# dfki-asr/morphablegraphs

Measured on AMD Instinct MI355X. Metric: motion-primitive samples scored+back-projected/sec; fraction of HBM roofline, higher is better.
Workload: dtype f32; 1 GPU; walk primitive L=40 F=156 D=79 NB=31 GMM k=8, batch=8192 candidates/GPU (BASELINE.json configs[1]); candidates_per_gpu=8192, global_candidates=8192, collective=none, clock_ramp_steps=1500

## Files before the change

### morphablegraphs_amd/csrc/mg_frames.hip

```cpp
#include "mg_frames_common.h"

int mg_setup_kernel_attributes(mg_context *) {
    int rc = mg_frames_ws_attributes();
    return rc != MG_OK ? rc : mg_frames_cs_attributes();
}

bool mg_frames_root_split(const mg_primitive *p) {
    const int want = p->ctx->opt[MG_OPT_ROOT_MODE];
    return want == 2 || (want == 3 && p->root_split);
}

static int mg_fused_gmm_lds(const mg_primitive *p) { return 4 * p->K * 16 * 8; }
static int mg_fused_gmm_lds_cs(const mg_primitive *p) {
    const int JT = (int)((p->Lg + 15) / 16);
    return mg_fused_gmm_lds(p) + 2 * p->KK * 64 * 4 + (p->K * JT * 16 + (p->K + 1) / 2 * 2) * 8;
}

static bool mg_fused_gmm_staged(const mg_primitive *p, const mg_time_grid *g) { return g->cs_lds_bytes + mg_fused_gmm_lds_cs(p) <= 160 * 1024; }

bool mg_frames_can_fuse_gmm(const mg_primitive *p, const mg_time_grid *g, int64_t B) {
    const int64_t n_tiles = (B + MG_NCAND - 1) / MG_NCAND;
    const int64_t grid = std::min<int64_t>(n_tiles * g->n_chunks, std::max(1, p->ctx->n_cu - p->ctx->reserved_cus));
    return g->mfma_ok && p->d_gPpack != nullptr && p->K <= 16 && p->KK <= MG_FUSE_MAX_KK && p->Lg == p->L &&
           g->lds_bytes + mg_fused_gmm_lds(p) <= 160 * 1024 &&
           (n_tiles + grid - 1) / grid <= 4;
}

int mg_frames_kernel_choice(const mg_primitive *p, const mg_time_grid *g, int64_t B, bool fused, const void *out, bool lat_f64) {
    const int64_t n_tiles = (B + MG_NCAND - 1) / MG_NCAND;
    const int64_t units = n_tiles * g->n_chunks;
    const int64_t grid0 = std::min<int64_t>(units, std::max(1, p->ctx->n_cu - p->ctx->reserved_cus));
    const int64_t grid_cs = grid0 / g->n_chunks * g->n_chunks;
    const int want = p->ctx->opt[MG_OPT_FRAMES_KERNEL];
    bool cs = g->cs_ok && grid_cs >= g->n_chunks && grid_cs <= 4096 &&
              (!fused || (g->cs_lds_bytes + mg_fused_gmm_lds(p) <= 160 * 1024 && (n_tiles + grid_cs - 1) / grid_cs <= 4));
    const bool cs_spills = p->KK >= 16 || (lat_f64 && p->KK >= 14);
    if (want == 2 && !cs) return -1;
    if (want == 1) cs = false;
    else if (want == 0 && cs_spills) cs = false;
    else if (want == 0) cs = cs && units >= 2 * grid0 && mg_output_class(p->ctx, out) != 0;
    return cs ? 2 : 1;
}
int mg_frames_grid(const mg_primitive *p, const mg_time_grid *g, int64_t B, int which) {
    const int64_t units = (B + MG_NCAND - 1) / MG_NCAND * g->n_chunks;
    const int64_t grid0 = std::min<int64_t>(units, std::max(1, p->ctx->n_cu - p->ctx->reserved_cus));
    return (int)(which == 2 ? grid0 / g->n_chunks * g->n_chunks : grid0);
}

int mg_frames_lds_bytes(const mg_primitive *p, const mg_time_grid *g, int which, bool fused) {
    if (which == 2) return g->cs_lds_bytes + (fused ? (mg_fused_gmm_staged(p, g) ? mg_fused_gmm_lds_cs(p) : mg_fused_gmm_lds(p)) : 0);
    return g->lds_bytes + (fused ? mg_fused_gmm_lds(p) : 0);
}

int mg_launch_frames_mfma(mg_primitive *p, const mg_time_grid *g, const void *lat, int ldt, int64_t B, int64_t ld, float *out, float *logp,
                          int prof_slot, int prof_slot2) {
    mg_frames_args a;
    a.rt_total = p->RT;
    a.B = B; a.ld = ld; a.T = g->T; a.D = p->D; a.Dp = p->Dp; a.cshift = p->cshift; a.L = p->L; a.nroot = p->nroot;
    a.n_chunks = g->n_chunks; a.stride = g->stride; a.max_wi = g->max_wi; a.max_nt = g->max_nt; a.nbuf = g->nbuf;
    const int64_t n_tiles = (B + MG_NCAND - 1) / MG_NCAND;
    const int64_t units = n_tiles * g->n_chunks;
    if (n_tiles >= ((int64_t)1 << 27) || units >= ((int64_t)1 << 31)) {
        mg_set_error("mg_back_project_frames: batch too large for one launch");
        return MG_ERR_UNSUPPORTED;
    }
    a.n_tiles = (int32_t)n_tiles;
    a.max_tiles = g->max_tiles;
    for (int i = 0; i < MG_ARG_CHUNKS; i++) a.ck[i] = i < g->n_chunks ? g->chunks[i] : mg_chunk{};
    a.cs_magic = a.cs_per = a.cs_rem = 0;
    const bool lf = (ldt == MG_F64);
    const int which = mg_frames_kernel_choice(p, g, B, logp != nullptr, out, lf);
    if (which < 0) {
        mg_set_error("mg_back_project_frames: the chunk-stationary kernel does not cover this shape (window of %d row tiles, %d bytes of LDS)",
                     g->max_tiles, g->cs_lds_bytes);
        return MG_ERR_UNSUPPORTED;
    }
    const bool cs = which == 2;
    const int buf_bytes = (MG_NCAND * g->stride * 4 + 255) / 256 * 256;
    int lds = g->nbuf * (buf_bytes + MG_RO_BYTES_N(g->max_nt) + MG_TB_BYTES_N(g->max_nt)) + MG_NCAND * (g->max_wi * p->nroot + 1) * 8 + 128;
    if (lds != g->lds_bytes || lds > 160 * 1024 || (logp && !mg_frames_can_fuse_gmm(p, g, B))) {
        mg_set_error("mg_back_project_frames: internal LDS sizing mismatch (%d vs %d)", lds, g->lds_bytes);
        return MG_ERR_UNSUPPORTED;
    }
    if (cs) lds = g->cs_lds_bytes;
    a.gmm_staged = cs && logp && mg_fused_gmm_staged(p, g) ? 1 : 0;
    if (logp) lds += a.gmm_staged ? mg_fused_gmm_lds_cs(p) : mg_fused_gmm_lds(p);
    const int grid = mg_frames_grid(p, g, B, which);
    if (cs) {
        const int Q = grid / g->n_chunks;
        a.cs_magic = (1 << 20) / g->n_chunks + 1;
        a.cs_per = (int32_t)(n_tiles / Q);
        a.cs_rem = (int32_t)(n_tiles % Q);
    }
    mg_launch_events ev;
    if (prof_slot >= 0) (void)mg_prof_kernel(p->ctx, prof_slot, prof_slot2, &ev.start, &ev.stop);
    const bool split = mg_frames_root_split(p);
    return cs ? mg_launch_frames_cs(p, g, lat, out, logp, a, lf, split, buf_bytes, lds, grid, ev)
              : mg_launch_frames_ws(p, g, lat, out, logp, a, lf, split, buf_bytes, lds, grid, ev);
}
```

### morphablegraphs_amd/csrc/mg_frames_common.h

```cpp
#pragma once
#include "mg_internal.h"
#include <hip/hip_ext.h>
#include <type_traits>
#include "mg_gmm_device.h"

typedef float f32x4 __attribute__((ext_vector_type(4)));
typedef double f64x4 __attribute__((ext_vector_type(4)));
typedef float f32x4u __attribute__((ext_vector_type(4), aligned(4)));
typedef float f32x3u __attribute__((ext_vector_type(3), aligned(4)));
typedef float f32x2u __attribute__((ext_vector_type(2), aligned(4)));

struct mg_frames_args {
    int64_t B, ld;
    int32_t T, D, Dp, cshift, L, nroot, n_chunks, n_tiles, stride, max_wi, max_nt;
    int32_t nbuf;
    int32_t max_tiles;
    int32_t rt_total;
    int32_t gmm_staged;
    int32_t cs_magic, cs_per, cs_rem;
    mg_chunk ck[MG_ARG_CHUNKS];
};

template <bool F64>
__device__ __forceinline__ double mg_load_lat(const void *lat, int64_t idx) {
// ... 153 lines not shown
        *(f32x4u *)op = v;
    } else if (n == 3) {
        f32x3u t = {v[0], v[1], v[2]};
        *(f32x3u *)op = t;
    } else if (n == 2) {
        f32x2u t = {v[0], v[1]};
        *(f32x2u *)op = t;
    } else if (n == 1) {
        op[0] = v[0];
    }
}


template <int KK>
__device__ __forceinline__ void mg_produce_f32(const float2 *__restrict__ ep, const float *__restrict__ mean32,
                                               const mg_chunk &ck, float *lds_c, int stride, int t_first, int pw, int npw,
                                               const float (&sfrag)[KK], int lane, int cl, int g, int rot = 0) {
    float2 fa[2][KK / 2], na[2][KK / 2];
    f32x4 fm[2], nm[2];
    auto load_tile = [&](int t, float2(&fr)[KK / 2], f32x4 &cin) {
        const int tc = t < ck.ntiles ? t : ck.ntiles - 1;
        const float2 *p = ep + ((size_t)(ck.rt0 + tc) * (KK / 2)) * 64 + lane;
#pragma unroll
        for (int q = 0; q < KK / 2; q++) fr[q] = p[q * 64];
        cin = *(const f32x4 *)(mean32 + (size_t)(ck.rt0 + tc) * 16 + 4 * g);
    };
    const int span = ck.ntiles - t_first - pw;
    const int nrounds = span > 0 ? (span + 2 * npw - 1) / (2 * npw) : 0;
    if (nrounds == 0) return;
    int rr = rot % nrounds;
    int t = t_first + pw + 2 * npw * rr;
    load_tile(t, fa[0], fm[0]);
    load_tile(t + npw, fa[1], fm[1]);
    for (int r = 0; r < nrounds; r++) {
        if (++rr == nrounds) rr = 0;
        const int tn = t_first + pw + 2 * npw * rr;
        load_tile(tn, na[0], nm[0]);
        load_tile(tn + npw, na[1], nm[1]);
        f32x4 acc0 = fm[0], acc1 = fm[1];
#pragma unroll
        for (int q = 0; q < KK / 2; q++) {
            acc0 = __builtin_amdgcn_mfma_f32_16x16x4f32(fa[0][q].x, sfrag[2 * q], acc0, 0, 0, 0);
            acc1 = __builtin_amdgcn_mfma_f32_16x16x4f32(fa[1][q].x, sfrag[2 * q], acc1, 0, 0, 0);
            acc0 = __builtin_amdgcn_mfma_f32_16x16x4f32(fa[0][q].y, sfrag[2 * q + 1], acc0, 0, 0, 0);
            acc1 = __builtin_amdgcn_mfma_f32_16x16x4f32(fa[1][q].y, sfrag[2 * q + 1], acc1, 0, 0, 0);
        }
        if (t < ck.ntiles) *(f32x4 *)&lds_c[cl * stride + t * 16 + 4 * g] = acc0;
        if (t + npw < ck.ntiles) *(f32x4 *)&lds_c[cl * stride + (t + npw) * 16 + 4 * g] = acc1;
#pragma unroll
        for (int q = 0; q < KK / 2; q++) { fa[0][q] = na[0][q]; fa[1][q] = na[1][q]; }
        fm[0] = nm[0]; fm[1] = nm[1];
        t = tn;
    }
}

template <int KK, bool LAT_F64>
__device__ __forceinline__ void mg_load_sfrag(float (&sfrag)[KK], const void *lat, const mg_unit &un, int64_t ld, int L, int cl, int g) {
    typename mg_gmm_xt<LAT_F64>::type x[KK];
    mg_gmm_load_x<KK, LAT_F64>(x, lat, un.b0, un.ncand, ld, L, cl, g);
#pragma unroll
    for (int kk = 0; kk < KK; kk++) sfrag[kk] = (float)x[kk];
}


template <int KK, bool LAT_F64>
__device__ __forceinline__ void mg_fused_gmm_terms(mg_lds_int *prog, const double *__restrict__ gPpack,
                                                   const double *__restrict__ gmP, const double *__restrict__ gcst,
                                                   const void *__restrict__ lat, int64_t B, int64_t ld, int L, int n_tiles,
                                                   int gK, int gJT, int pw, int lane, int group) {
    const int cl = lane & 15, g = lane >> 4;
    mg_lds_f64 *gterms = (mg_lds_f64 *)(prog + 32);
    const int64_t gt0 = (int64_t)blockIdx.x * n_tiles / gridDim.x + 2 * group;
    const int64_t gt1 = ((int64_t)blockIdx.x + 1) * n_tiles / gridDim.x;
    if (gt0 < gt1) {
        const bool has_b = gt0 + 1 < gt1;
        typename mg_gmm_xt<LAT_F64>::type xa[KK], xb[KK];
        {
            const int64_t ba = gt0 * MG_NCAND, bb = (has_b ? gt0 + 1 : gt0) * MG_NCAND;
            const int na = (int)((B - ba) < MG_NCAND ? (B - ba) : MG_NCAND);
            const int nb = (int)((B - bb) < MG_NCAND ? (B - bb) : MG_NCAND);
            mg_gmm_load_x<KK, LAT_F64>(xa, lat, ba, na, ld, L, cl, g);
            mg_gmm_load_x<KK, LAT_F64>(xb, lat, bb, nb, ld, L, cl, g);
        }
        for (int k = pw; k < gK; k += MG_WS_NPW) {
            mg_gmm_frag<KK> f;
            mg_gmm_load_component<KK>(f, gPpack, gmP, gcst, k, gJT, lane, cl, gK);
            mg_gmm_apply_component(f, k, gJT, xa, gterms, cl, g);
            if (has_b) mg_gmm_apply_component(f, k, gJT, xb, gterms + gK * 16, cl, g);
        }
    }
    mg_publish(prog + 16, pw, lane, group + 1);
}

template <int KK>
__device__ __forceinline__ void mg_fused_gmm_terms_ldsx(mg_lds_int *prog, const double *__restrict__ gPpack, const mg_lds_f32 *gx, const mg_lds_f64 *mpl,
                                                        const mg_lds_f64 *cstl, int n_tiles, int gK, int gJT, int pw, int lane, bool early) {
    const int cl = lane & 15, g = lane >> 4;
    mg_lds_f64 *gterms = (mg_lds_f64 *)(prog + 32);
    const int64_t gt0 = (int64_t)blockIdx.x * n_tiles / gridDim.x;
    const int64_t gt1 = ((int64_t)blockIdx.x + 1) * n_tiles / gridDim.x;
    if (gt0 < gt1) {
        const bool has_b = gt0 + 1 < gt1;
        int ks[4], nk = 0;
        for (int k = pw; k < gK; k += MG_WS_NPW)
            if (!(early && k >= MG_WS_NPW && k < 2 * MG_WS_NPW)) ks[nk++] = k;
        for (int i = 0; i < nk; i += 2) {
            const int k = ks[i], k2 = i + 1 < nk ? ks[i + 1] : gK;
            mg_gmm_frag<KK> f, f2;
            mg_gmm_load_pf2<KK>(f, gPpack, gK, k, gJT, lane);
            if (k2 < gK) mg_gmm_load_pf2<KK>(f2, gPpack, gK, k2, gJT, lane);
            mg_gmm_apply_component_ldsx<KK>(f, k, gJT, gx, lane, mpl, cstl, gterms, cl, g);
            if (has_b) mg_gmm_apply_component_ldsx<KK>(f, k, gJT, gx + KK * 64, lane, mpl, cstl, gterms + gK * 16, cl, g);
            if (k2 < gK) {
                mg_gmm_apply_component_ldsx<KK>(f2, k2, gJT, gx, lane, mpl, cstl, gterms, cl, g);
                if (has_b) mg_gmm_apply_component_ldsx<KK>(f2, k2, gJT, gx + KK * 64, lane, mpl, cstl, gterms + gK * 16, cl, g);
            }
        }
    }
    mg_publish(prog + 16, pw, lane, 1);
}

template <int KK>
__device__ __forceinline__ void mg_fused_gmm_early_component(mg_lds_int *prog, const mg_gmm_frag<KK> &f, int k, const mg_lds_f32 *gx, const mg_lds_f64 *mpl,
                                                             const mg_lds_f64 *cstl, int n_tiles, int gK, int gJT, int lane) {
    const int cl = lane & 15, g = lane >> 4;
    mg_lds_f64 *gterms = (mg_lds_f64 *)(prog + 32);
    const int64_t gt0 = (int64_t)blockIdx.x * n_tiles / gridDim.x;
    const int64_t gt1 = ((int64_t)blockIdx.x + 1) * n_tiles / gridDim.x;
    mg_gmm_apply_component_ldsx<KK>(f, k, gJT, gx, lane, mpl, cstl, gterms, cl, g);
    if (gt0 + 1 < gt1) mg_gmm_apply_component_ldsx<KK>(f, k, gJT, gx + KK * 64, lane, mpl, cstl, gterms + gK * 16, cl, g);
}

__device__ __forceinline__ void mg_fused_gmm_finish(mg_lds_int *prog, float *__restrict__ logp, int64_t B, int n_tiles, int gK,
                                                    int pw, int lane, int group) {
    mg_lds_int *gdone = prog + 16;
    mg_lds_f64 *gterms = (mg_lds_f64 *)(prog + 32);
    mg_lds_f64 *gexps = gterms + 2 * gK * 16;
    const int64_t gt0 = (int64_t)blockIdx.x * n_tiles / gridDim.x + 2 * group;
    const int64_t gt1 = ((int64_t)blockIdx.x + 1) * n_tiles / gridDim.x;
    if (pw < 2 && gt0 + pw < gt1) {
        mg_wait_producers(gdone, group + 1);
        const mg_lds_f64 *terms = gterms + pw * gK * 16;
        mg_lds_f64 *exps = gexps + pw * gK * 16;
        for (int e = lane; e < gK * 16; e += 64) exps[e] = mg_gmm_exp_entry(terms, gK, e);
        asm volatile("s_waitcnt lgkmcnt(0)" ::: "memory");
        const int64_t b0 = (gt0 + pw) * MG_NCAND;
        if (lane < MG_NCAND && b0 + lane < B) logp[b0 + lane] = (float)mg_gmm_logsumexp(terms, exps, gK, lane);
    }
    if (pw < 2) mg_publish(prog + 24, pw, lane, group + 1);
}


struct mg_launch_events { hipEvent_t start = nullptr, stop = nullptr; };
int mg_launch_frames_ws(mg_primitive *p, const mg_time_grid *g, const void *lat, float *out, float *logp, const mg_frames_args &a, bool lat_f64,
                        bool split, int buf_bytes, int lds, int grid, const mg_launch_events &ev);
int mg_launch_frames_cs(mg_primitive *p, const mg_time_grid *g, const void *lat, float *out, float *logp, const mg_frames_args &a, bool lat_f64,
                        bool split, int buf_bytes, int lds, int grid, const mg_launch_events &ev);
int mg_frames_ws_attributes();
int mg_frames_cs_attributes();
```

### morphablegraphs_amd/csrc/mg_frames_cs.hip

```cpp
#include "mg_frames_common.h"

#define MG_CS_NPW 4
#define MG_CS_NCW 8
#define MG_CS_NSP 4
#define MG_CS_BLOCK (64 * (MG_CS_NPW + MG_CS_NCW))
template <int KK> struct mg_cs_cfg {
    static constexpr int TPWP = 120 / KK < 17 ? 120 / KK : 17;
    static constexpr int TPWS_REGS = 160 / MG_CS_NSP;
    static constexpr int TPWS = TPWS_REGS / KK < 5 ? (TPWS_REGS / KK > 0 ? TPWS_REGS / KK : 1) : 5;
    static constexpr int MAX_TILES = (MG_CS_NPW - 1) * TPWP + MG_CS_NSP * TPWS;
};
int mg_cs_max_tiles(int KK) {
    switch (KK) {
        case 2: return mg_cs_cfg<2>::MAX_TILES;   case 4: return mg_cs_cfg<4>::MAX_TILES;   case 6: return mg_cs_cfg<6>::MAX_TILES;
        case 8: return mg_cs_cfg<8>::MAX_TILES;   case 10: return mg_cs_cfg<10>::MAX_TILES; case 12: return mg_cs_cfg<12>::MAX_TILES;
        case 14: return mg_cs_cfg<14>::MAX_TILES; case 16: return mg_cs_cfg<16>::MAX_TILES; default: return 0;
    }
}

#define MG_CS_PROG_LAT 12
#define MG_CS_PROG_SWEPT 16
#define MG_CS_PROG_MEAN 24
#define MG_CS_PROG_GMM 32
#define MG_CS_PROG_INTS 64
// ... 487 lines not shown
        int tap_b_off[3][MG_TAP_KS], tap_o_off[3], rs_off[3][4];
#pragma unroll
        for (int ct = 0; ct < 3; ct++) {
            const int col = ct * 16 + cl;
            const bool colok = col < MG_NCAND * nroot;
            const int cc = colok ? col / nroot : 0, cd = colok ? col - cc * nroot : 0;
            tap_o_off[ct] = colok ? cc * MG_RO_CS(max_nt) + cd : 3;
#pragma unroll
            for (int ks = 0; ks < MG_TAP_KS; ks++) {
                const int m = 4 * ks + g;
                tap_b_off[ct][ks] = (colok && m < ck.wi) ? cc * root_stride + m * nroot + cd : rs_zero;
            }
        }
#pragma unroll
        for (int t = 0; t < 3; t++) {
            const int lr0 = (ck.rrt0 + t) * 16 + g - ck.imin * nroot;
#pragma unroll
            for (int r = 0; r < 4; r++) {
                const int lr = lr0 + 4 * r;
                rs_off[t][r] = cl * root_stride + ((t < ck.nrt && lr >= 0 && lr < ck.wi * nroot) ? lr : a.max_wi * nroot);
            }
        }
        auto park_tables = [&]() {
            float4 *tw = (float4 *)tb_base;
            int *tmo = (int *)(tw + max_nt);
#pragma unroll
            for (int e = 0; e < MG_TAP_FT * MG_TAP_KS; e++) lds_rwt[e * 64 + lane] = wt_v[e];
            if (lane < ck.nT) {
                tw[lane] = tw_v;
                tmo[lane] = (ti_v - ck.imin) * Dp * 4;
            }
        };
        if (lane == 63) lds_rmean[63] = 0.0;
        auto root_unit = [&](const int u, auto first_tag) {
            constexpr bool FIRST = decltype(first_tag)::value;
#pragma unroll
            for (int kk = 0; kk < KK; kk++) s64frag[kk] = s64next[kk];
            if (u >= 2) mg_cs_wait_swept(prog, u - 1);
            {
                float *lb = lds_latb + (u & 1) * KK * 64;
#pragma unroll
                for (int kk = 0; kk < KK; kk++) lb[kk * 64 + lane] = (float)s64frag[kk];
                mg_publish(prog, MG_CS_PROG_LAT, lane, u + 1);
            }
            if (!FIRST) load_latents(s64next, u + 1);
            f64x4 racc[3];
#pragma unroll
            for (int t = 0; t < 3; t++) {
                if (FIRST) {
                    racc[t] = f64x4{rm_v[t][0], rm_v[t][1], rm_v[t][2], rm_v[t][3]};
                    if (cl == 0) {
#pragma unroll
                        for (int r = 0; r < 4; r++) lds_rmean[(t * 4 + r) * 4 + g] = rm_v[t][r];
                    }
                } else {
                    racc[t] = f64x4{lds_rmean[(t * 4 + 0) * 4 + g], lds_rmean[(t * 4 + 1) * 4 + g], lds_rmean[(t * 4 + 2) * 4 + g], lds_rmean[(t * 4 + 3) * 4 + g]};
                }
            }
            if (RR) {
#pragma unroll
                for (int q2 = 0; q2 < KK; q2++)
#pragma unroll
                    for (int t = 0; t < 3; t++)
                        racc[t] = __builtin_amdgcn_mfma_f64_16x16x4f64(rp_reg[t][RR ? q2 : 0], (double)s64frag[q2], racc[t], 0, 0, 0);
            } else {
                constexpr int CH = KK <= 12 ? KK / 2 : 4;
#pragma unroll
                for (int h0 = 0; h0 < KK; h0 += CH) {
                    double rp[3][CH];
#pragma unroll
                    for (int t = 0; t < 3; t++)
#pragma unroll
                        for (int q2 = 0; q2 < CH; q2++) rp[t][q2] = rpp[t][(h0 + q2 < KK ? h0 + q2 : KK - 1) * 64];
#pragma unroll
                    for (int q2 = 0; q2 < CH; q2++)
#pragma unroll
                        for (int t = 0; t < 3; t++)
                            if (h0 + q2 < KK) racc[t] = __builtin_amdgcn_mfma_f64_16x16x4f64(rp[t][q2], (double)s64frag[h0 + q2 < KK ? h0 + q2 : KK - 1], racc[t], 0, 0, 0);
                }
            }
#pragma unroll
            for (int t = 0; t < 3; t++)
#pragma unroll
                for (int r = 0; r < 4; r++) rs[rs_off[t][r]] = racc[t][r];
            if (FIRST) park_tables();
            float *ro = (float *)(ro_base + (size_t)(u & 1) * RO_BYTES);
            double bv[3][MG_TAP_KS];
#pragma unroll
            for (int ct = 0; ct < 3; ct++)
#pragma unroll
                for (int ks = 0; ks < MG_TAP_KS; ks++) bv[ct][ks] = rs[tap_b_off[ct][ks]];
#pragma unroll
            for (int ft = 0; ft < MG_TAP_FT; ft++) {
                if (ft * 16 < ck.nT) {
                    f64x4 acc[3];
#pragma unroll
                    for (int ct = 0; ct < 3; ct++) acc[ct] = {0.0, 0.0, 0.0, 0.0};
#pragma unroll
                    for (int ks = 0; ks < MG_TAP_KS; ks++)
#pragma unroll
                        for (int ct = 0; ct < 3; ct++)
                            acc[ct] = __builtin_amdgcn_mfma_f64_16x16x4f64(lds_rwt[(ft * MG_TAP_KS + ks) * 64 + lane], bv[ct][ks], acc[ct], 0, 0, 0);
#pragma unroll
                    for (int ct = 0; ct < 3; ct++)
#pragma unroll
                        for (int r = 0; r < 4; r++) ro[tap_o_off[ct] + (ft * 16 + g + 4 * r) * 4] = (float)acc[ct][r];
                }
            }
            mg_publish(prog, wave, lane, u + 1);
            if (FIRST) load_latents(s64next, 1);
        };
        if (n_units > 0) root_unit(0, std::true_type{});
        for (int u = 1; u < n_units; u++) root_unit(u, std::false_type{});
        }
    }
    if (FUSE_GMM && wave < MG_WS_NPW) {
        mg_lds_int *gprog = prog + MG_CS_PROG_GMM;
        bool staged = false;
        if constexpr (GMM_LDSX) staged = a.gmm_staged != 0;
        if (staged) {
            if constexpr (GMM_LDSX) {
                mg_wait_producers(gprog + 20, 1);
                mg_fused_gmm_terms_ldsx<KK>(gprog, gPpack, mg_cs_gmm_x(prog, gK), mg_cs_gmm_mp(prog, gK, KK), mg_cs_gmm_mp(prog, gK, KK) + gK * gJT * 16,
                                            a.n_tiles, gK, gJT, wave, lane, GMM_HALF && mg_cs_gmm_early(a));
                if constexpr (GMM_HALF) mg_wait_producers(gprog + 28, 1);
            }
        } else
            mg_fused_gmm_terms<KK, LAT_F64>(gprog, gPpack, gmP, gcst, lat, a.B, a.ld, L, a.n_tiles, gK, gJT, wave, lane, 0);
        if (wave < 2) mg_fused_gmm_finish(gprog, logp, a.B, a.n_tiles, gK, wave, lane, 0);
        const int64_t my_tiles = ((int64_t)blockIdx.x + 1) * a.n_tiles / gridDim.x - (int64_t)blockIdx.x * a.n_tiles / gridDim.x;
        if (my_tiles > 2) {
            mg_wait_producers(gprog + 24, 1);
            mg_fused_gmm_terms<KK, LAT_F64>(gprog, gPpack, gmP, gcst, lat, a.B, a.ld, L, a.n_tiles, gK, gJT, wave, lane, 1);
            if (wave < 2) mg_fused_gmm_finish(gprog, logp, a.B, a.n_tiles, gK, wave, lane, 1);
        }
    }
}


template <int KK, bool LAT_F64, bool FUSE, bool SPLIT>
static int mg_launch_cs_inst(mg_primitive *p, const mg_time_grid *g, const void *lat, float *out, float *logp, const mg_frames_args &a,
                                 int buf_bytes, int lds, int grid, const mg_launch_events &ev) {
    hipExtLaunchKernelGGL((mg_frames_cs_kernel<KK, LAT_F64, FUSE, SPLIT>), dim3(grid), dim3(MG_CS_BLOCK), lds, p->ctx->stream, ev.start, ev.stop, 0,
                          (const float *)p->d_Epack, (const float *)p->d_mean32, (const double *)p->d_Erpack, (const double *)p->d_meanroot, lat,
                          (const int32_t *)g->d_i0, (const float4 *)g->d_w32, (const double *)g->d_wtap, (const float4 *)g->d_rootm,
                          (const mg_chunk *)g->d_chunks, out,
                          (const double *)p->d_gPpack, (const double *)p->d_gmPpad, (const double *)p->d_gconst, logp, a, (int)p->K,
                          (int)((p->L + 15) / 16), buf_bytes);
    MG_HIP_CHECK(hipGetLastError());
    return MG_OK;
}

template <int KK>
static int mg_launch_cs_kk(mg_primitive *p, const mg_time_grid *g, const void *lat, float *out, float *logp, const mg_frames_args &a,
                               bool lat_f64, bool split, int buf_bytes, int lds, int grid, const mg_launch_events &ev) {
    if (logp) {
        if constexpr (KK <= MG_FUSE_MAX_KK) {
            if (split)
                return lat_f64 ? mg_launch_cs_inst<KK, true, true, true>(p, g, lat, out, logp, a, buf_bytes, lds, grid, ev)
                               : mg_launch_cs_inst<KK, false, true, true>(p, g, lat, out, logp, a, buf_bytes, lds, grid, ev);
            return lat_f64 ? mg_launch_cs_inst<KK, true, true, false>(p, g, lat, out, logp, a, buf_bytes, lds, grid, ev)
                           : mg_launch_cs_inst<KK, false, true, false>(p, g, lat, out, logp, a, buf_bytes, lds, grid, ev);
        }
        mg_set_error("mg_step_frames_and_logp: no fused kernel for %d components", p->L);
        return MG_ERR_UNSUPPORTED;
    }
    if (split)
        return lat_f64 ? mg_launch_cs_inst<KK, true, false, true>(p, g, lat, out, nullptr, a, buf_bytes, lds, grid, ev)
                       : mg_launch_cs_inst<KK, false, false, true>(p, g, lat, out, nullptr, a, buf_bytes, lds, grid, ev);
    return lat_f64 ? mg_launch_cs_inst<KK, true, false, false>(p, g, lat, out, nullptr, a, buf_bytes, lds, grid, ev)
                   : mg_launch_cs_inst<KK, false, false, false>(p, g, lat, out, nullptr, a, buf_bytes, lds, grid, ev);
}

int mg_launch_frames_cs(mg_primitive *p, const mg_time_grid *g, const void *lat, float *out, float *logp, const mg_frames_args &a, bool lat_f64,
                        bool split, int buf_bytes, int lds, int grid, const mg_launch_events &ev) {
    switch (p->KK) {
        case 2: return mg_launch_cs_kk<2>(p, g, lat, out, logp, a, lat_f64, split, buf_bytes, lds, grid, ev);
        case 4: return mg_launch_cs_kk<4>(p, g, lat, out, logp, a, lat_f64, split, buf_bytes, lds, grid, ev);
        case 6: return mg_launch_cs_kk<6>(p, g, lat, out, logp, a, lat_f64, split, buf_bytes, lds, grid, ev);
        case 8: return mg_launch_cs_kk<8>(p, g, lat, out, logp, a, lat_f64, split, buf_bytes, lds, grid, ev);
        case 10: return mg_launch_cs_kk<10>(p, g, lat, out, logp, a, lat_f64, split, buf_bytes, lds, grid, ev);
        case 12: return mg_launch_cs_kk<12>(p, g, lat, out, logp, a, lat_f64, split, buf_bytes, lds, grid, ev);
        case 14: return mg_launch_cs_kk<14>(p, g, lat, out, logp, a, lat_f64, split, buf_bytes, lds, grid, ev);
        case 16: return mg_launch_cs_kk<16>(p, g, lat, out, logp, a, lat_f64, split, buf_bytes, lds, grid, ev);
        default: mg_set_error("mg_back_project_frames: MFMA path needs n_components <= 64"); return MG_ERR_UNSUPPORTED;
    }
}

template <int KK>
static int mg_cs_attr_kk() {
    MG_HIP_CHECK(hipFuncSetAttribute((const void *)mg_frames_cs_kernel<KK, true, false, false>, hipFuncAttributeMaxDynamicSharedMemorySize, 160 * 1024));
    MG_HIP_CHECK(hipFuncSetAttribute((const void *)mg_frames_cs_kernel<KK, false, false, false>, hipFuncAttributeMaxDynamicSharedMemorySize, 160 * 1024));
    MG_HIP_CHECK(hipFuncSetAttribute((const void *)mg_frames_cs_kernel<KK, true, false, true>, hipFuncAttributeMaxDynamicSharedMemorySize, 160 * 1024));
    MG_HIP_CHECK(hipFuncSetAttribute((const void *)mg_frames_cs_kernel<KK, false, false, true>, hipFuncAttributeMaxDynamicSharedMemorySize, 160 * 1024));
    if constexpr (KK <= MG_FUSE_MAX_KK) {
        MG_HIP_CHECK(hipFuncSetAttribute((const void *)mg_frames_cs_kernel<KK, true, true, false>, hipFuncAttributeMaxDynamicSharedMemorySize, 160 * 1024));
        MG_HIP_CHECK(hipFuncSetAttribute((const void *)mg_frames_cs_kernel<KK, false, true, false>, hipFuncAttributeMaxDynamicSharedMemorySize, 160 * 1024));
        MG_HIP_CHECK(hipFuncSetAttribute((const void *)mg_frames_cs_kernel<KK, true, true, true>, hipFuncAttributeMaxDynamicSharedMemorySize, 160 * 1024));
        MG_HIP_CHECK(hipFuncSetAttribute((const void *)mg_frames_cs_kernel<KK, false, true, true>, hipFuncAttributeMaxDynamicSharedMemorySize, 160 * 1024));
    }
    return MG_OK;
}
int mg_frames_cs_attributes() {
    int rc;
    if ((rc = mg_cs_attr_kk<2>()) != MG_OK) return rc;
    if ((rc = mg_cs_attr_kk<4>()) != MG_OK) return rc;
    if ((rc = mg_cs_attr_kk<6>()) != MG_OK) return rc;
    if ((rc = mg_cs_attr_kk<8>()) != MG_OK) return rc;
    if ((rc = mg_cs_attr_kk<10>()) != MG_OK) return rc;
    if ((rc = mg_cs_attr_kk<12>()) != MG_OK) return rc;
    if ((rc = mg_cs_attr_kk<14>()) != MG_OK) return rc;
    if ((rc = mg_cs_attr_kk<16>()) != MG_OK) return rc;
    return MG_OK;
}
```

### morphablegraphs_amd/csrc/mg_frames_ws.hip

```cpp
#include "mg_frames_common.h"

template <int KK, bool LAT_F64, bool FUSE_GMM, bool SPLIT>
__global__ __launch_bounds__(MG_WS_BLOCK) void mg_frames_ws_kernel(
    const float *__restrict__ Epack,
    const float *__restrict__ mean32,
    const double *__restrict__ Erpack,
    const double *__restrict__ meanroot,
    const void *__restrict__ lat,
    const int32_t *__restrict__ i0tab,
    const float4 *__restrict__ w32,
    const double *__restrict__ wtap,
    const float4 *__restrict__ rootm,
    const mg_chunk *__restrict__ chunks,
    float *__restrict__ out,
    const double *__restrict__ gPpack,
    const double *__restrict__ gmP,
    const double *__restrict__ gcst,
    float *__restrict__ logp,
    const mg_frames_args a, const int gK, const int gJT, const int buf_bytes) {
    extern __shared__ __attribute__((aligned(16))) unsigned char smem[];
    const int tid = threadIdx.x;
    const int lane = tid & 63;
    const int wave = __builtin_amdgcn_readfirstlane(tid >> 6);
    const int stride = a.stride, D = a.D, Dp = a.Dp, L = a.L, nroot = a.nroot;
// ... 218 lines not shown
            prev_tile = un.tile;
            prev_chunk = un.chunk;
            mg_publish(prog, wave, lane, u + 1);
            if (++slot == nbuf) slot = 0;
        }
    } else {
        int tap_b_off[3][MG_TAP_KS], tap_o_off[3];
        bool tap_b_ok[3][MG_TAP_KS];
#pragma unroll
        for (int ct = 0; ct < 3; ct++) {
            const int col = ct * 16 + cl;
            const bool colok = col < MG_NCAND * nroot;
            const int cc = colok ? col / nroot : 0, cd = colok ? col - cc * nroot : 0;
            tap_o_off[ct] = colok ? cc * MG_RO_CS(max_nt) + cd : -1;
#pragma unroll
            for (int ks = 0; ks < MG_TAP_KS; ks++) {
                const int m = 4 * ks + g;
                tap_b_ok[ct][ks] = colok && m < a.max_wi;
                tap_b_off[ct][ks] = cc * root_stride + m * nroot + cd;
            }
        }
        auto root_stage = [&](const mg_unit &un, int slot) {
            const mg_chunk &ck = un.ck;
            float4 *tw = (float4 *)(tb_base + (size_t)slot * MG_TB_BYTES);
            int *tmo = (int *)(tw + max_nt);
            double *rs = (double *)rs_base;
            float4 r_w = {0.f, 0.f, 0.f, 0.f};
            int r_i0 = 0;
            if (lane < ck.nT) { r_w = w32[ck.t0 + lane]; r_i0 = i0tab[ck.t0 + lane]; }
            if constexpr (SPLIT) {
                float4 *tm = (float4 *)(ro_base + (size_t)slot * MG_RO_BYTES);
                if (lane < ck.nT) {
                    const float4 mh = rootm[2 * (ck.t0 + lane)], ml = rootm[2 * (ck.t0 + lane) + 1];
                    tw[lane] = r_w;
                    tmo[lane] = (r_i0 - ck.imin) * Dp * 4;
                    tm[2 * lane] = mh;
                    tm[2 * lane + 1] = ml;
                }
                return;
            }
            double r_wt[MG_TAP_FT * MG_TAP_KS];
#pragma unroll
            for (int e = 0; e < MG_TAP_FT * MG_TAP_KS; e++) r_wt[e] = wtap[((size_t)un.chunk * (MG_TAP_FT * MG_TAP_KS) + e) * 64 + lane];
            typename mg_gmm_xt<LAT_F64>::type s64frag[KK];
            mg_gmm_load_x<KK, LAT_F64>(s64frag, lat, un.b0, un.ncand, a.ld, L, cl, g);
            f64x4 racc[3];
            const double *rpp[3];
#pragma unroll
            for (int t = 0; t < 3; t++) {
                const int tc = t < ck.nrt ? t : ck.nrt - 1;
                rpp[t] = Erpack + ((size_t)(ck.rrt0 + tc) * KK) * 64 + lane;
                const int row0 = (ck.rrt0 + tc) * 16;
                racc[t][0] = meanroot[row0 + g];
                racc[t][1] = meanroot[row0 + g + 4];
                racc[t][2] = meanroot[row0 + g + 8];
                racc[t][3] = meanroot[row0 + g + 12];
            }
            constexpr int NH = KK <= 10 ? 1 : 2;
            constexpr int KH = KK / NH;
#pragma unroll
            for (int h = 0; h < NH; h++) {
                double rp[3][KH];
#pragma unroll
                for (int t = 0; t < 3; t++)
#pragma unroll
                    for (int q = 0; q < KH; q++) rp[t][q] = rpp[t][(h * KH + q) * 64];
                if (h == 0) {
                    if (lane < ck.nT) {
                        tw[lane] = r_w;
                        tmo[lane] = (r_i0 - ck.imin) * Dp * 4;
                    }
                }
#pragma unroll
                for (int q = 0; q < KH; q++)
#pragma unroll
                    for (int t = 0; t < 3; t++)
                        racc[t] = __builtin_amdgcn_mfma_f64_16x16x4f64(rp[t][q], (double)s64frag[h * KH + q], racc[t], 0, 0, 0);
            }
#pragma unroll
            for (int t = 0; t < 3; t++) {
                const int lr0 = (ck.rrt0 + t) * 16 + g - ck.imin * nroot;
#pragma unroll
                for (int r = 0; r < 4; r++) {
                    const int lr = lr0 + 4 * r;
                    if (t < ck.nrt && lr >= 0 && lr < ck.wi * nroot) rs[cl * root_stride + lr] = racc[t][r];
                }
            }
            float *ro = (float *)(ro_base + (size_t)slot * MG_RO_BYTES);
#pragma unroll
            for (int ft = 0; ft < MG_TAP_FT; ft++) {
                if (ft * 16 < ck.nT) {
                    f64x4 acc[3];
                    double bv[3][MG_TAP_KS];
#pragma unroll
                    for (int ct = 0; ct < 3; ct++) {
                        acc[ct] = {0.0, 0.0, 0.0, 0.0};
#pragma unroll
                        for (int ks = 0; ks < MG_TAP_KS; ks++)
                            bv[ct][ks] = (tap_b_ok[ct][ks] && 4 * ks + g < ck.wi) ? rs[tap_b_off[ct][ks]] : 0.0;
                    }
#pragma unroll
                    for (int ks = 0; ks < MG_TAP_KS; ks++)
#pragma unroll
                        for (int ct = 0; ct < 3; ct++)
                            acc[ct] = __builtin_amdgcn_mfma_f64_16x16x4f64(r_wt[ft * MG_TAP_KS + ks], bv[ct][ks], acc[ct], 0, 0, 0);
#pragma unroll
                    for (int ct = 0; ct < 3; ct++)
#pragma unroll
                        for (int r = 0; r < 4; r++) {
                            const int fo = ft * 16 + g + 4 * r;
                            if (tap_o_off[ct] >= 0 && fo < ck.nT) ro[tap_o_off[ct] + fo * 4] = (float)acc[ct][r];
                        }
                }
            }
        };
        int slot = 0;
        for (int u = 0; u < n_units; u++) {
            const mg_unit un = mg_unit_at(chunks, a, cur, rot);
            mg_cursor_next(cur, a.n_chunks);
            if (u >= nbuf) mg_wait_consumers(prog, u - nbuf + 1);
            root_stage(un, slot);
            mg_publish(prog, wave, lane, u + 1);
            if (++slot == nbuf) slot = 0;
        }
    }
    if (FUSE_GMM && wave < MG_WS_NPW) {
        mg_fused_gmm_terms<KK, LAT_F64>(prog, gPpack, gmP, gcst, lat, a.B, a.ld, L, a.n_tiles, gK, gJT, wave, lane, 0);
        if (wave < 2) mg_fused_gmm_finish(prog, logp, a.B, a.n_tiles, gK, wave, lane, 0);
        const int64_t my_tiles = ((int64_t)blockIdx.x + 1) * a.n_tiles / gridDim.x - (int64_t)blockIdx.x * a.n_tiles / gridDim.x;
        if (my_tiles > 2) {
            mg_wait_producers(prog + 24, 1);
            mg_fused_gmm_terms<KK, LAT_F64>(prog, gPpack, gmP, gcst, lat, a.B, a.ld, L, a.n_tiles, gK, gJT, wave, lane, 1);
            if (wave < 2) mg_fused_gmm_finish(prog, logp, a.B, a.n_tiles, gK, wave, lane, 1);
        }
    }
}



template <int KK, bool LAT_F64, bool FUSE, bool SPLIT>
static int mg_launch_ws_inst(mg_primitive *p, const mg_time_grid *g, const void *lat, float *out, float *logp, const mg_frames_args &a,
                                 int buf_bytes, int lds, int grid, const mg_launch_events &ev) {
    hipExtLaunchKernelGGL((mg_frames_ws_kernel<KK, LAT_F64, FUSE, SPLIT>), dim3(grid), dim3(MG_WS_BLOCK), lds, p->ctx->stream, ev.start, ev.stop, 0,
                          (const float *)p->d_Epack, (const float *)p->d_mean32, (const double *)p->d_Erpack, (const double *)p->d_meanroot, lat,
                          (const int32_t *)g->d_i0, (const float4 *)g->d_w32, (const double *)g->d_wtap, (const float4 *)g->d_rootm,
                          (const mg_chunk *)g->d_chunks, out,
                          (const double *)p->d_gPpack, (const double *)p->d_gmPpad, (const double *)p->d_gconst, logp, a, (int)p->K,
                          (int)((p->L + 15) / 16), buf_bytes);
    MG_HIP_CHECK(hipGetLastError());
    return MG_OK;
}

template <int KK>
static int mg_launch_ws_kk(mg_primitive *p, const mg_time_grid *g, const void *lat, float *out, float *logp, const mg_frames_args &a,
                               bool lat_f64, bool split, int buf_bytes, int lds, int grid, const mg_launch_events &ev) {
    if (logp) {
        if constexpr (KK <= MG_FUSE_MAX_KK) {
            if (split)
                return lat_f64 ? mg_launch_ws_inst<KK, true, true, true>(p, g, lat, out, logp, a, buf_bytes, lds, grid, ev)
                               : mg_launch_ws_inst<KK, false, true, true>(p, g, lat, out, logp, a, buf_bytes, lds, grid, ev);
            return lat_f64 ? mg_launch_ws_inst<KK, true, true, false>(p, g, lat, out, logp, a, buf_bytes, lds, grid, ev)
                           : mg_launch_ws_inst<KK, false, true, false>(p, g, lat, out, logp, a, buf_bytes, lds, grid, ev);
        }
        mg_set_error("mg_step_frames_and_logp: no fused kernel for %d components", p->L);
        return MG_ERR_UNSUPPORTED;
    }
    if (split)
        return lat_f64 ? mg_launch_ws_inst<KK, true, false, true>(p, g, lat, out, nullptr, a, buf_bytes, lds, grid, ev)
                       : mg_launch_ws_inst<KK, false, false, true>(p, g, lat, out, nullptr, a, buf_bytes, lds, grid, ev);
    return lat_f64 ? mg_launch_ws_inst<KK, true, false, false>(p, g, lat, out, nullptr, a, buf_bytes, lds, grid, ev)
                   : mg_launch_ws_inst<KK, false, false, false>(p, g, lat, out, nullptr, a, buf_bytes, lds, grid, ev);
}

int mg_launch_frames_ws(mg_primitive *p, const mg_time_grid *g, const void *lat, float *out, float *logp, const mg_frames_args &a, bool lat_f64,
                        bool split, int buf_bytes, int lds, int grid, const mg_launch_events &ev) {
    switch (p->KK) {
        case 2: return mg_launch_ws_kk<2>(p, g, lat, out, logp, a, lat_f64, split, buf_bytes, lds, grid, ev);
        case 4: return mg_launch_ws_kk<4>(p, g, lat, out, logp, a, lat_f64, split, buf_bytes, lds, grid, ev);
        case 6: return mg_launch_ws_kk<6>(p, g, lat, out, logp, a, lat_f64, split, buf_bytes, lds, grid, ev);
        case 8: return mg_launch_ws_kk<8>(p, g, lat, out, logp, a, lat_f64, split, buf_bytes, lds, grid, ev);
        case 10: return mg_launch_ws_kk<10>(p, g, lat, out, logp, a, lat_f64, split, buf_bytes, lds, grid, ev);
        case 12: return mg_launch_ws_kk<12>(p, g, lat, out, logp, a, lat_f64, split, buf_bytes, lds, grid, ev);
        case 14: return mg_launch_ws_kk<14>(p, g, lat, out, logp, a, lat_f64, split, buf_bytes, lds, grid, ev);
        case 16: return mg_launch_ws_kk<16>(p, g, lat, out, logp, a, lat_f64, split, buf_bytes, lds, grid, ev);
        default: mg_set_error("mg_back_project_frames: MFMA path needs n_components <= 64"); return MG_ERR_UNSUPPORTED;
    }
}

template <int KK>
static int mg_ws_attr_kk() {
    MG_HIP_CHECK(hipFuncSetAttribute((const void *)mg_frames_ws_kernel<KK, true, false, false>, hipFuncAttributeMaxDynamicSharedMemorySize, 160 * 1024));
    MG_HIP_CHECK(hipFuncSetAttribute((const void *)mg_frames_ws_kernel<KK, false, false, false>, hipFuncAttributeMaxDynamicSharedMemorySize, 160 * 1024));
    MG_HIP_CHECK(hipFuncSetAttribute((const void *)mg_frames_ws_kernel<KK, true, false, true>, hipFuncAttributeMaxDynamicSharedMemorySize, 160 * 1024));
    MG_HIP_CHECK(hipFuncSetAttribute((const void *)mg_frames_ws_kernel<KK, false, false, true>, hipFuncAttributeMaxDynamicSharedMemorySize, 160 * 1024));
    if constexpr (KK <= MG_FUSE_MAX_KK) {
        MG_HIP_CHECK(hipFuncSetAttribute((const void *)mg_frames_ws_kernel<KK, true, true, false>, hipFuncAttributeMaxDynamicSharedMemorySize, 160 * 1024));
        MG_HIP_CHECK(hipFuncSetAttribute((const void *)mg_frames_ws_kernel<KK, false, true, false>, hipFuncAttributeMaxDynamicSharedMemorySize, 160 * 1024));
        MG_HIP_CHECK(hipFuncSetAttribute((const void *)mg_frames_ws_kernel<KK, true, true, true>, hipFuncAttributeMaxDynamicSharedMemorySize, 160 * 1024));
        MG_HIP_CHECK(hipFuncSetAttribute((const void *)mg_frames_ws_kernel<KK, false, true, true>, hipFuncAttributeMaxDynamicSharedMemorySize, 160 * 1024));
    }
    return MG_OK;
}
int mg_frames_ws_attributes() {
    int rc;
    if ((rc = mg_ws_attr_kk<2>()) != MG_OK) return rc;
    if ((rc = mg_ws_attr_kk<4>()) != MG_OK) return rc;
    if ((rc = mg_ws_attr_kk<6>()) != MG_OK) return rc;
    if ((rc = mg_ws_attr_kk<8>()) != MG_OK) return rc;
    if ((rc = mg_ws_attr_kk<10>()) != MG_OK) return rc;
    if ((rc = mg_ws_attr_kk<12>()) != MG_OK) return rc;
    if ((rc = mg_ws_attr_kk<14>()) != MG_OK) return rc;
    if ((rc = mg_ws_attr_kk<16>()) != MG_OK) return rc;
    return MG_OK;
}
```

### morphablegraphs_amd/csrc/mg_host.hip

```cpp
#include <algorithm>
#include <cmath>
#include <cstdarg>
#include <cstdio>
#include <cstdlib>
#include <cstring>
#include <new>
#include <time.h>

#include "mg_internal.h"
#include <dlfcn.h>

static thread_local char g_err[1024] = "";

void mg_set_error(const char *fmt, ...) {
    va_list ap;
    va_start(ap, fmt);
    vsnprintf(g_err, sizeof(g_err), fmt, ap);
    va_end(ap);
}

int mg_hip_fail(hipError_t e, const char *what) {
    mg_set_error("HIP error %d (%s) in %s", (int)e, hipGetErrorString(e), what);
    if (e == hipErrorOutOfMemory) return MG_ERR_OUT_OF_MEMORY;
    if (e == hipErrorNoDevice || e == hipErrorInvalidDevice) return MG_ERR_NO_DEVICE;
    return MG_ERR_HIP;
}

extern "C" const char *mg_version(void) { return "mg_hip 0.1 (gfx950)"; }
extern "C" const char *mg_last_error(void) { return g_err; }
extern "C" const char *mg_status_string(int s) {
    switch (s) {
        case MG_OK: return "ok";
        case MG_ERR_INVALID_ARGUMENT: return "invalid argument";
        case MG_ERR_NO_DEVICE: return "no HIP device";
        case MG_ERR_HIP: return "HIP runtime error";
        case MG_ERR_UNSUPPORTED: return "unsupported shape";
        case MG_ERR_NOT_POSITIVE_DEFINITE: return "covariance not positive definite";
        case MG_ERR_OUT_OF_MEMORY: return "out of device memory";
        default: return "unknown status";
    }
}

#define MG_REQUIRE(cond, ...) MG_REQUIRE_AS(cond, MG_ERR_INVALID_ARGUMENT, __VA_ARGS__)

struct mg_nccl_id { char internal[MG_DIST_ID_BYTES]; };
struct mg_rccl_api {
    void *lib = nullptr;
    int (*GetUniqueId)(void *) = nullptr;
    int (*CommInitRank)(void **, int,  mg_nccl_id, int) = nullptr;
    int (*AllGather)(const void *, void *, size_t, int, void *, hipStream_t) = nullptr;
    int (*Broadcast)(const void *, void *, size_t, int, int, void *, hipStream_t) = nullptr;
    int (*CommDestroy)(void *) = nullptr;
    const char *(*GetErrorString)(int) = nullptr;
};
static mg_rccl_api g_rccl;
static int mg_rccl_load() {
    if (g_rccl.lib) return MG_OK;
    void *h = dlopen("librccl.so.1", RTLD_NOW | RTLD_LOCAL);
    if (!h) h = dlopen("librccl.so", RTLD_NOW | RTLD_LOCAL);
    if (!h) { mg_set_error("mg_dist: librccl.so.1 cannot be loaded (%s)", dlerror()); return MG_ERR_UNSUPPORTED; }
    g_rccl.GetUniqueId = (int (*)(void *))dlsym(h, "ncclGetUniqueId");
    g_rccl.CommInitRank = (int (*)(void **, int, mg_nccl_id, int))dlsym(h, "ncclCommInitRank");
    g_rccl.AllGather = (int (*)(const void *, void *, size_t, int, void *, hipStream_t))dlsym(h, "ncclAllGather");
    g_rccl.Broadcast = (int (*)(const void *, void *, size_t, int, int, void *, hipStream_t))dlsym(h, "ncclBroadcast");
    g_rccl.CommDestroy = (int (*)(void *))dlsym(h, "ncclCommDestroy");
    g_rccl.GetErrorString = (const char *(*)(int))dlsym(h, "ncclGetErrorString");
    if (!g_rccl.GetUniqueId || !g_rccl.CommInitRank || !g_rccl.AllGather || !g_rccl.Broadcast || !g_rccl.CommDestroy) {
        mg_set_error("mg_dist: librccl lacks an expected symbol");
        dlclose(h);
        return MG_ERR_UNSUPPORTED;
    }
    g_rccl.lib = h;
    return MG_OK;
}
static int mg_rccl_fail(int rc, const char *what) {
    mg_set_error("RCCL error %d (%s) in %s", rc, g_rccl.GetErrorString ? g_rccl.GetErrorString(rc) : "?", what);
    return MG_ERR_HIP;
}
__attribute__((constructor)) static void mg_runtime_settings() { (void)setenv("HIP_FORCE_DEV_KERNARG", "1", 0); }

extern "C" int mg_context_create(int device, void *stream, mg_context **out) {
    MG_REQUIRE(out != nullptr, "mg_context_create: out is NULL");
    *out = nullptr;
    int n = 0;
    hipError_t e = hipGetDeviceCount(&n);
    if (e != hipSuccess || n <= 0) {
        mg_set_error("mg_context_create: no HIP device available (%s)", e == hipSuccess ? "count = 0" : hipGetErrorString(e));
        return MG_ERR_NO_DEVICE;
    }
    MG_REQUIRE(device >= 0 && device < n, "mg_context_create: device %d out of range [0,%d)", device, n);
    MG_HIP_CHECK(hipSetDevice(device));
    mg_context *ctx = new (std::nothrow) mg_context();
    if (!ctx) return MG_ERR_OUT_OF_MEMORY;
    ctx->device = device;
    hipDeviceProp_t prop;
    e = hipGetDeviceProperties(&prop, device);
    if (e != hipSuccess) { delete ctx; return mg_hip_fail(e, "hipGetDeviceProperties"); }
    ctx->n_cu = prop.multiProcessorCount;
    ctx->total_mem = (int64_t)prop.totalGlobalMem;
    ctx->max_lds = (int)prop.maxSharedMemoryPerMultiProcessor;
    snprintf(ctx->name, sizeof(ctx->name), "%s (%s, %d CUs)", prop.name[0] ? prop.name : "AMD Instinct", prop.gcnArchName, prop.multiProcessorCount);
    if (strncmp(prop.gcnArchName, "gfx950", 6) != 0) {
        mg_set_error("mg_context_create: device %d is %s; this library is built for gfx950 only", device, prop.gcnArchName);
        delete ctx;
        return MG_ERR_UNSUPPORTED;
    }
    if (stream) {
        ctx->stream = (hipStream_t)stream;
        ctx->own_stream = false;
    } else {
        e = hipStreamCreateWithFlags(&ctx->stream, hipStreamNonBlocking);
        if (e != hipSuccess) { delete ctx; return mg_hip_fail(e, "hipStreamCreate"); }
        ctx->own_stream = true;
    }
    e = hipMalloc(&ctx->argmin_out, 16);
    if (e != hipSuccess) { mg_context_destroy(ctx); return mg_hip_fail(e, "hipMalloc"); }
    int rc = mg_setup_kernel_attributes(ctx);
    if (rc == MG_OK) rc = mg_options_fused_attributes();
    if (rc != MG_OK) { mg_context_destroy(ctx); return rc; }
    *out = ctx;
    return MG_OK;
}

static void mg_vmm_release(mg_context *ctx, mg_context::vmm_alloc &v);
extern "C" void mg_context_destroy(mg_context *ctx) {
    if (!ctx) return;
    (void)hipSetDevice(ctx->device);
    (void)hipStreamSynchronize(ctx->stream);
    if (ctx->rccl_comm && g_rccl.CommDestroy) { (void)g_rccl.CommDestroy(ctx->rccl_comm); ctx->rccl_comm = nullptr; }
    for (auto &p : ctx->pending) { (void)hipEventDestroy(p.a); (void)hipEventDestroy(p.b); }
    for (auto &ev : ctx->free_events) (void)hipEventDestroy(ev);
    for (auto &st : ctx->side) if (st) (void)hipStreamDestroy(st);
    for (auto &e : ctx->side_ev) if (e) (void)hipEventDestroy(e);
    if (ctx->scratch) (void)mg_device_free(ctx, ctx->scratch);
    mg_output_release_all(ctx);
    if (ctx->argmin_out) (void)hipFree(ctx->argmin_out);
    for (void *q : {ctx->fused_tab_dev, ctx->fused_counters, ctx->fused_partials, ctx->fused_dyn_dev}) if (q) (void)hipFree(q);
    if (ctx->pinned) (void)hipHostFree(ctx->pinned);
    if (ctx->flag_block) (void)hipHostFree(ctx->flag_block);
    if (ctx->traj_paths) (void)hipFree(ctx->traj_paths);
    if (ctx->lists_dev) (void)hipFree(ctx->lists_dev);
    if (ctx->tree_tab_dev) (void)hipFree(ctx->tree_tab_dev);
    if (ctx->walk_tab_dev) (void)hipFree(ctx->walk_tab_dev);
    if (ctx->wscore_tab_dev) (void)hipFree(ctx->wscore_tab_dev);
    if (ctx->wtime_tab_dev) (void)hipFree(ctx->wtime_tab_dev);
    if (ctx->slen_tab_dev) (void)hipFree(ctx->slen_tab_dev);
    for (auto &b : ctx->arena) (void)hipFree(b.base);
    for (auto &v : ctx->vmm) mg_vmm_release(ctx, v);
    (void)hipDeviceSynchronize();
    for (auto &r : ctx->vmm_parked) (void)hipMemAddressFree(r.first, r.second);
    ctx->vmm_parked.clear();
    if (ctx->own_stream && ctx->stream) (void)hipStreamDestroy(ctx->stream);
    delete ctx;
}

extern "C" int mg_context_set_stream(mg_context *ctx, void *stream) {
    MG_REQUIRE(ctx != nullptr, "mg_context_set_stream: ctx is NULL");
    MG_HIP_CHECK(hipStreamSynchronize(ctx->stream));
    if (ctx->own_stream && ctx->stream) (void)hipStreamDestroy(ctx->stream);
    if (stream) {
        ctx->stream = (hipStream_t)stream;
        ctx->own_stream = false;
    } else {
        MG_HIP_CHECK(hipStreamCreateWithFlags(&ctx->stream, hipStreamNonBlocking));
        ctx->own_stream = true;
    }
    return MG_OK;
}

extern "C" int mg_context_arena_begin(mg_context *ctx, int64_t block_bytes) {
    MG_REQUIRE(ctx != nullptr && block_bytes >= 0, "mg_context_arena_begin: bad arguments");
    ctx->arena_block_bytes = block_bytes > 0 ? (size_t)block_bytes : ((size_t)64 << 20);
    return MG_OK;
}
extern "C" int mg_context_arena_end(mg_context *ctx) {
    MG_REQUIRE(ctx != nullptr, "mg_context_arena_end: ctx is NULL");
    ctx->arena_block_bytes = 0;
    return MG_OK;
}
extern "C" int mg_context_arena_bytes(mg_context *ctx, int64_t *reserved, int64_t *used) {
    MG_REQUIRE(ctx != nullptr, "mg_context_arena_bytes: ctx is NULL");
    int64_t r = 0, u = 0;
    for (auto &b : ctx->arena) { r += (int64_t)b.bytes; u += (int64_t)b.used; }
    if (reserved) *reserved = r;
    if (used) *used = u;
    return MG_OK;
}
static int mg_arena_alloc(mg_context *ctx, size_t bytes, void **out) {
    const size_t need = (bytes + 255) / 256 * 256;
    if (ctx->arena.empty() || ctx->arena.back().used + need > ctx->arena.back().bytes) {
        mg_context::arena_block b;
        b.bytes = std::max(ctx->arena_block_bytes, need);
        b.used = 0;
        b.live = 0;
        MG_HIP_CHECK(hipMalloc((void **)&b.base, b.bytes));
        ctx->arena.push_back(b);
    }
    *out = ctx->arena.back().base + ctx->arena.back().used;
    ctx->arena.back().used += need;
    ctx->arena.back().live++;
    return MG_OK;
}
void mg_dev_free(mg_context *ctx, void *p) {
    if (!p) return;
    for (size_t i = 0; i < ctx->arena.size(); i++) {
        mg_context::arena_block &b = ctx->arena[i];
        if ((char *)p >= b.base && (char *)p < b.base + b.bytes) {
            if (--b.live == 0 && !(ctx->arena_block_bytes > 0 && i + 1 == ctx->arena.size())) {
                (void)hipFree(b.base);
                ctx->arena.erase(ctx->arena.begin() + (long)i);
            }
            return;
        }
    }
    (void)hipFree(p);
}

extern "C" int mg_dist_unique_id(void *id_out) {
    MG_REQUIRE(id_out != nullptr, "mg_dist_unique_id: id_out is NULL");
    int rc = mg_rccl_load();
    if (rc != MG_OK) return rc;
    int nrc = g_rccl.GetUniqueId(id_out);
    return nrc == 0 ? MG_OK : mg_rccl_fail(nrc, "ncclGetUniqueId");
}
extern "C" int mg_dist_preflight(mg_context *ctx) {
    MG_REQUIRE(ctx != nullptr, "mg_dist_preflight: ctx is NULL");
    int rc = mg_rccl_load();
    if (rc != MG_OK) return rc;
    MG_HIP_CHECK(hipSetDevice(ctx->device));
    MG_HIP_CHECK(hipStreamSynchronize(ctx->stream));
    return MG_OK;
}
extern "C" int mg_dist_info(mg_context *ctx, int32_t *out3) {
    MG_REQUIRE(ctx && out3, "mg_dist_info: NULL argument");
    out3[0] = -1; out3[1] = 0; out3[2] = -1;
    if (!ctx->rccl_comm || !g_rccl.lib) return MG_OK;
    typedef int (*q_fn)(void *, int *);
    const char *names[3] = {"ncclCommUserRank", "ncclCommCount", "ncclCommCuDevice"};
    for (int i = 0; i < 3; i++) {
        q_fn f = (q_fn)dlsym(g_rccl.lib, names[i]);
        int v = -1;
        if (f && f(ctx->rccl_comm, &v) == 0) out3[i] = v; else out3[i] = -1;
    }
    return MG_OK;
}
extern "C" int mg_dist_init(mg_context *ctx, int32_t rank, int32_t n_ranks, const void *id) {
    MG_REQUIRE(ctx && id && n_ranks >= 1 && rank >= 0 && rank < n_ranks, "mg_dist_init: bad arguments");
    MG_REQUIRE(ctx->rccl_comm == nullptr, "mg_dist_init: the context already has a communicator");
    int rc = mg_rccl_load();
    if (rc != MG_OK) return rc;
    MG_HIP_CHECK(hipSetDevice(ctx->device));
    mg_nccl_id uid;
    memcpy(uid.internal, id, MG_DIST_ID_BYTES);
    int nrc = g_rccl.CommInitRank(&ctx->rccl_comm, n_ranks, uid, rank);
    if (nrc != 0) { ctx->rccl_comm = nullptr; return mg_rccl_fail(nrc, "ncclCommInitRank"); }
    ctx->dist_rank = rank;
    ctx->dist_ranks = n_ranks;
    return MG_OK;
}
extern "C" int mg_dist_all_gather(mg_context *ctx, const void *local_dev, void *gathered_dev, int64_t count, int dtype) {
    MG_REQUIRE(ctx && count >= 0 && (count == 0 || (local_dev && gathered_dev)), "mg_dist_all_gather: bad arguments");
    MG_REQUIRE(dtype == MG_F32 || dtype == MG_F64, "mg_dist_all_gather: bad dtype %d", dtype);
    MG_REQUIRE(ctx->rccl_comm != nullptr, "mg_dist_all_gather: mg_dist_init has not been called on this context");
    if (count == 0) return MG_OK;
    MG_HIP_CHECK(hipSetDevice(ctx->device));
    int nrc = g_rccl.AllGather(local_dev, gathered_dev, (size_t)count, dtype == MG_F64 ? 8  : 7 ,
                               ctx->rccl_comm, ctx->stream);
    return nrc == 0 ? MG_OK : mg_rccl_fail(nrc, "ncclAllGather");
}
extern "C" int mg_dist_broadcast(mg_context *ctx, void *buf_dev, int64_t bytes, int32_t root) {
    MG_REQUIRE(ctx && ctx->rccl_comm, "mg_dist_broadcast: mg_dist_init has not been called on this context");
    MG_REQUIRE(bytes >= 0 && (bytes == 0 || buf_dev) && root >= 0 && root < ctx->dist_ranks, "mg_dist_broadcast: bad arguments");
    if (bytes == 0) return MG_OK;
    MG_HIP_CHECK(hipSetDevice(ctx->device));
    const int rcb = g_rccl.Broadcast(buf_dev, buf_dev, (size_t)bytes, 0 , root, ctx->rccl_comm, ctx->stream);
    return rcb == 0 ? MG_OK : mg_rccl_fail(rcb, "ncclBroadcast");
}
extern "C" int mg_dist_finalize(mg_context *ctx) {
    MG_REQUIRE(ctx != nullptr, "mg_dist_finalize: ctx is NULL");
    if (!ctx->rccl_comm) return MG_OK;
    MG_HIP_CHECK(hipStreamSynchronize(ctx->stream));
    int nrc = g_rccl.CommDestroy(ctx->rccl_comm);
    ctx->rccl_comm = nullptr;
    ctx->dist_rank = 0; ctx->dist_ranks = 1;
    return nrc == 0 ? MG_OK : mg_rccl_fail(nrc, "ncclCommDestroy");
}

extern "C" int mg_context_synchronize(mg_context *ctx) {
    MG_REQUIRE(ctx != nullptr, "mg_context_synchronize: ctx is NULL");
    MG_HIP_CHECK(hipStreamSynchronize(ctx->stream));
    return MG_OK;
}

extern "C" int mg_context_set_reserved_cus(mg_context *ctx, int32_t n) {
    MG_REQUIRE(ctx != nullptr && n >= 0, "mg_context_set_reserved_cus: bad arguments");
    ctx->reserved_cus = std::min<int32_t>(n, ctx->n_cu - 1);
    return MG_OK;
}
extern "C" int mg_context_set_option(mg_context *ctx, int32_t option, int32_t value) {
    MG_REQUIRE(ctx != nullptr, "mg_context_set_option: ctx is NULL");
    MG_REQUIRE(option >= 0 && option < MG_OPT_COUNT, "mg_context_set_option: unknown option %d", option);
    MG_REQUIRE(value >= 0, "mg_context_set_option: value %d < 0", value);
    ctx->opt[option] = value;
    return MG_OK;
}
extern "C" int mg_context_device_info(mg_context *ctx, char *name, int32_t *n_cu, int64_t *total_mem) {
    MG_REQUIRE(ctx != nullptr, "mg_context_device_info: ctx is NULL");
    if (name) { strncpy(name, ctx->name, 255); name[255] = 0; }
    if (n_cu) *n_cu = ctx->n_cu;
    if (total_mem) *total_mem = ctx->total_mem;
    return MG_OK;
}

extern "C" int mg_device_malloc(mg_context *ctx, int64_t bytes, void **out_dev) {
    MG_REQUIRE(ctx && out_dev && bytes >= 0, "mg_device_malloc: bad arguments");
    *out_dev = nullptr;
    MG_HIP_CHECK(hipSetDevice(ctx->device));
    if (bytes == 0) bytes = 16;
    if (bytes >= MG_PLACED_MIN_BYTES && !ctx->opt[MG_OPT_PLAIN_MALLOC]) return mg_output_alloc(ctx, bytes, 0, out_dev, nullptr);
    MG_HIP_CHECK(hipMalloc(out_dev, (size_t)bytes));
    return MG_OK;
}
static void mg_vmm_release(mg_context *ctx, mg_context::vmm_alloc &v) {
    if (v.va) {
        (void)hipMemUnmap(v.va, v.total);
        ctx->vmm_parked.push_back({v.va, v.total});
    }
    for (auto h : v.handles) (void)hipMemRelease(h);
    v.handles.clear();
    v.va = nullptr;
}
extern "C" int mg_device_malloc_chunked(mg_context *ctx, int64_t bytes, int64_t chunk_bytes, void **out_dev) {
    MG_REQUIRE(ctx && out_dev && bytes > 0 && chunk_bytes > 0, "mg_device_malloc_chunked: bad arguments");
    *out_dev = nullptr;
    MG_HIP_CHECK(hipSetDevice(ctx->device));
    hipMemAllocationProp prop = {};
    prop.type = hipMemAllocationTypePinned;
    prop.location.type = hipMemLocationTypeDevice;
    prop.location.id = ctx->device;
    size_t gran = 0;
    MG_HIP_CHECK(hipMemGetAllocationGranularity(&gran, &prop, hipMemAllocationGranularityMinimum));
    if (gran == 0) gran = 4096;
    const size_t chunk = ((size_t)chunk_bytes + gran - 1) / gran * gran;
    const size_t n = ((size_t)bytes + chunk - 1) / chunk;
    mg_context::vmm_alloc v;
    v.total = n * chunk; v.chunk = chunk; v.va = nullptr;
    hipError_t e = hipMemAddressReserve(&v.va, v.total, 0, nullptr, 0);
    if (e != hipSuccess) return mg_hip_fail(e, "hipMemAddressReserve");
    size_t mapped = 0;
    for (size_t i = 0; i < n && e == hipSuccess; i++) {
        hipMemGenericAllocationHandle_t h;
        e = hipMemCreate(&h, chunk, &prop, 0);
        if (e != hipSuccess) break;
        v.handles.push_back(h);
        e = hipMemMap((char *)v.va + i * chunk, chunk, 0, h, 0);
        if (e == hipSuccess) mapped += chunk;
    }
    if (e == hipSuccess) {
        hipMemAccessDesc acc = {};
        acc.location = prop.location;
        acc.flags = hipMemAccessFlagsProtReadWrite;
        e = hipMemSetAccess(v.va, v.total, &acc, 1);
    }
    if (e != hipSuccess) {
        if (mapped) (void)hipMemUnmap(v.va, mapped);
        (void)hipMemAddressFree(v.va, v.total);
        for (auto h : v.handles) (void)hipMemRelease(h);
        return mg_hip_fail(e, "mg_device_malloc_chunked (virtual-memory API)");
    }
    *out_dev = v.va;
    ctx->vmm.push_back(std::move(v));
    return MG_OK;
}
extern "C" int mg_device_free(mg_context *ctx, void *p) {
    MG_REQUIRE(ctx != nullptr, "mg_device_free: ctx is NULL");
    if (!p) return MG_OK;
    MG_HIP_CHECK(hipStreamSynchronize(ctx->stream));
    if (mg_output_free(ctx, p)) return MG_OK;
    return mg_device_free_raw(ctx, p);
}
int mg_device_free_raw(mg_context *ctx, void *p) {
    for (size_t i = 0; i < ctx->vmm.size(); i++)
        if (ctx->vmm[i].va == p) {
            mg_vmm_release(ctx, ctx->vmm[i]);
            ctx->vmm.erase(ctx->vmm.begin() + (long)i);
            return MG_OK;
        }
    MG_HIP_CHECK(hipFree(p));
    return MG_OK;
}
extern "C" int mg_memcpy_h2d(mg_context *ctx, void *dst, const void *src, int64_t bytes) {
    MG_REQUIRE(ctx && (bytes == 0 || (dst && src)) && bytes >= 0, "mg_memcpy_h2d: bad arguments");
    if (bytes == 0) return MG_OK;
    MG_HIP_CHECK(hipMemcpyAsync(dst, src, (size_t)bytes, hipMemcpyHostToDevice, ctx->stream));
    MG_HIP_CHECK(hipStreamSynchronize(ctx->stream));
    return MG_OK;
}
extern "C" int mg_memcpy_d2h(mg_context *ctx, void *dst, const void *src, int64_t bytes) {
    MG_REQUIRE(ctx && (bytes == 0 || (dst && src)) && bytes >= 0, "mg_memcpy_d2h: bad arguments");
    if (bytes == 0) return MG_OK;
    MG_HIP_CHECK(hipMemcpyAsync(dst, src, (size_t)bytes, hipMemcpyDeviceToHost, ctx->stream));
    MG_HIP_CHECK(hipStreamSynchronize(ctx->stream));
    return MG_OK;
}
extern "C" int mg_memset(mg_context *ctx, void *dst, int value, int64_t bytes) {
    MG_REQUIRE(ctx && (bytes == 0 || dst) && bytes >= 0, "mg_memset: bad arguments");
    if (bytes == 0) return MG_OK;
    MG_HIP_CHECK(hipMemsetAsync(dst, value, (size_t)bytes, ctx->stream));
    return MG_OK;
}

int mg_ctx_scratch(mg_context *ctx, int64_t bytes, void **out) {
    if (bytes > ctx->scratch_bytes) {
        MG_HIP_CHECK(hipStreamSynchronize(ctx->stream));
        if (ctx->scratch) { int rcf = mg_device_free(ctx, ctx->scratch); ctx->scratch = nullptr; ctx->scratch_bytes = 0; if (rcf != MG_OK) return rcf; }
        int64_t want = std::max<int64_t>(bytes, 1 << 20);
        int rcm = mg_device_malloc(ctx, want, &ctx->scratch);
        if (rcm != MG_OK) return rcm;
        ctx->scratch_bytes = want;
    }
    *out = ctx->scratch;
    return MG_OK;
}

static hipEvent_t mg_get_event(mg_context *ctx) {
    if (!ctx->free_events.empty()) {
        hipEvent_t e = ctx->free_events.back();
        ctx->free_events.pop_back();
        return e;
    }
    hipEvent_t e = nullptr;
    (void)hipEventCreateWithFlags(&e, hipEventDisableSystemFence);
    return e;
}
void mg_prof_begin(mg_context *ctx, int slot) {
    if (!ctx->profile) return;
    if (ctx->prof_interval > 1 && (ctx->prof_seen[slot]++ % ctx->prof_interval) != 0) return;
    if (ctx->pending.size() > 4096) (void)mg_prof_resolve(ctx);
    mg_event_pair p;
    p.a = mg_get_event(ctx);
    p.b = mg_get_event(ctx);
    p.slot = slot;
    p.ended = false;
    (void)hipEventRecord(p.a, ctx->stream);
    ctx->pending.push_back(p);
}
bool mg_prof_kernel(mg_context *ctx, int slot, int slot2, hipEvent_t *start, hipEvent_t *stop) {
    if (!ctx->profile) return false;
    if (ctx->prof_interval > 1 && (ctx->prof_seen[slot]++ % ctx->prof_interval) != 0) return false;
    if (ctx->pending.size() > 4096) (void)mg_prof_resolve(ctx);
    mg_event_pair p;
    p.a = mg_get_event(ctx);
    p.b = mg_get_event(ctx);
    p.slot = slot;
    p.slot2 = slot2;
    p.ended = true;
    ctx->pending.push_back(p);
    *start = p.a;
    *stop = p.b;
    return true;
}
void mg_prof_end(mg_context *ctx, int slot) {
    if (!ctx->profile) return;
    for (size_t i = ctx->pending.size(); i-- > 0;) {
        mg_event_pair &p = ctx->pending[i];
        if (p.slot == slot && !p.ended) {
            (void)hipEventRecord(p.b, ctx->stream);
            p.ended = true;
            return;
        }
    }
}
int mg_prof_resolve(mg_context *ctx) {
    for (auto &p : ctx->pending) {
        float ms = 0.f;
        if (p.ended && hipEventSynchronize(p.b) == hipSuccess && hipEventElapsedTime(&ms, p.a, p.b) == hipSuccess) {
            for (int sl : {p.slot, p.slot2}) {
                if (sl < 0) continue;
                ctx->prof_ms[sl] += (double)ms;
                ctx->prof_n[sl] += 1;
                if (ctx->prof_samples[sl].size() < 65536) ctx->prof_samples[sl].push_back(ms);
            }
        }
        ctx->free_events.push_back(p.a);
        ctx->free_events.push_back(p.b);
    }
    ctx->pending.clear();
    return MG_OK;
}
extern "C" int mg_profile_enable(mg_context *ctx, int enabled) {
    MG_REQUIRE(ctx != nullptr, "mg_profile_enable: ctx is NULL");
    if (!enabled) (void)mg_prof_resolve(ctx);
    ctx->profile = enabled != 0;
    ctx->prof_interval = enabled > 1 ? enabled : 1;
    for (int i = 0; i < MG_PROFILE_SLOTS; i++) ctx->prof_seen[i] = 0;
    return MG_OK;
}
extern "C" int mg_profile_reset(mg_context *ctx) {
    MG_REQUIRE(ctx != nullptr, "mg_profile_reset: ctx is NULL");
    (void)mg_prof_resolve(ctx);
    for (int i = 0; i < MG_PROFILE_SLOTS; i++) { ctx->prof_ms[i] = 0; ctx->prof_n[i] = 0; ctx->prof_samples[i].clear(); }
    return MG_OK;
}
extern "C" int mg_profile_get(mg_context *ctx, int slot, double *total_ms, int64_t *launches) {
    MG_REQUIRE(ctx && slot >= 0 && slot < MG_PROFILE_SLOTS, "mg_profile_get: bad arguments");
    (void)mg_prof_resolve(ctx);
    if (total_ms) *total_ms = ctx->prof_ms[slot];
    if (launches) *launches = ctx->prof_n[slot];
    return MG_OK;
}
extern "C" int mg_profile_get_samples(mg_context *ctx, int slot, float *out_ms, int64_t capacity, int64_t *n) {
    MG_REQUIRE(ctx && slot >= 0 && slot < MG_PROFILE_SLOTS && capacity >= 0 && (capacity == 0 || out_ms) && n,
               "mg_profile_get_samples: bad arguments");
    (void)mg_prof_resolve(ctx);
    const std::vector<float> &v = ctx->prof_samples[slot];
    const int64_t m = std::min<int64_t>(capacity, (int64_t)v.size());
    for (int64_t i = 0; i < m; i++) out_ms[i] = v[(size_t)i];
    *n = m;
    return MG_OK;
}

void mg_basis_row(const double *t, int n, double x, int32_t *i0, double *h) {
    const int k = 3;
    int l = k;
    while (!(x < t[l + 1] || l == n - k - 2)) l++;
    double hh[4];
    h[0] = 1.0; h[1] = h[2] = h[3] = 0.0;
    for (int j = 1; j <= k; j++) {
        for (int i = 0; i < j; i++) hh[i] = h[i];
        h[0] = 0.0;
        for (int i = 1; i <= j; i++) {
            int li = l + i, lj = li - j;
            if (t[li] == t[lj]) { h[i] = 0.0; continue; }
            double f = hh[i - 1] / (t[li] - t[lj]);
            h[i - 1] = h[i - 1] + f * (t[li] - x);
            h[i] = f * (x - t[lj]);
        }
    }
    *i0 = l - k;
}

static bool mg_cholesky_lower(const double *S, int L, double *c) {
    std::fill(c, c + (size_t)L * L, 0.0);
    for (int j = 0; j < L; j++) {
        double sum = S[j * L + j];
        for (int p = 0; p < j; p++) sum -= c[j * L + p] * c[j * L + p];
        if (!(sum > 0.0) || !std::isfinite(sum)) return false;
        c[j * L + j] = std::sqrt(sum);
        for (int i = j + 1; i < L; i++) {
            double s2 = S[i * L + j];
            for (int p = 0; p < j; p++) s2 -= c[i * L + p] * c[j * L + p];
            c[i * L + j] = s2 / c[j * L + j];
        }
// ... 67 lines not shown
            a0 = b;
        }
        return n;
    };
    int W = 0, best_n = 0;
    for (int w = MG_MAX_WI; w >= 4; w--) {
        if (!fits(w, budget1)) continue;
        const int n = count_chunks(w);
        if (W == 0 || n <= best_n) { W = w; best_n = n; }
    }
    if (W == 0) return;
    if (const int o = p->ctx->opt[MG_OPT_CHUNK_WINDOW]) W = std::max(4, std::min(W, o));
    const int n_greedy = count_chunks(W);
    int a = 0;
    int max_stride = 0, max_wi = 0, longest = 0;
    while (a < g->T) {
        int imin = g->i0[a], imax = g->i0[a];
        int b = a + 1;
        const int left = std::max(1, n_greedy - (int)g->chunks.size());
        const int target = std::min(max_nt, (g->T - a + left - 1) / left);
        while (b < g->T && b - a < target) {
            int lo = std::min(imin, g->i0[b]), hi = std::max(imax, g->i0[b]);
            if (hi - lo + 4 > W) break;
            imin = lo; imax = hi;
            b++;
        }
        mg_chunk c;
        memset(&c, 0, sizeof(c));
        c.t0 = a;
        c.nT = b - a;
        c.imin = imin;
        c.wi = imax - imin + 4;
        c.rt0 = (imin * Dp) / 16;
        int rt1 = ((imin + c.wi) * Dp + 15) / 16;
        c.ntiles = rt1 - c.rt0;
        c.rrt0 = (imin * p->nroot) / 16;
        c.nrt = ((imin + c.wi) * p->nroot + 15) / 16 - c.rrt0;
        g->chunks.push_back(c);
        max_stride = std::max(max_stride, mg_round_stride(c.ntiles * 16));
        max_wi = std::max(max_wi, c.wi);
        longest = std::max(longest, c.nT);
        a = b;
    }
    g->stride = max_stride;
    g->max_wi = max_wi;
    g->max_nt = (longest + 15) / 16 * 16;
    g->nbuf = mg_lds_bytes(p, max_stride, max_wi, 3, g->max_nt) <= budget1 ? 3 : 2;
    if (p->ctx->opt[MG_OPT_RING_SLOTS] == 2) g->nbuf = 2;
    g->lds_bytes = mg_lds_bytes(p, max_stride, max_wi, g->nbuf, g->max_nt);
    g->n_chunks = (int32_t)g->chunks.size();
    g->mfma_ok = g->lds_bytes <= budget1;
    g->max_tiles = 0;
    for (const mg_chunk &c : g->chunks) g->max_tiles = std::max(g->max_tiles, c.ntiles);
    {
        const int buf = (MG_NCAND * max_stride * 4 + 255) / 256 * 256;
        g->cs_lds_bytes = 2 * (buf + MG_RO_BYTES_N(g->max_nt)) + g->max_nt * 20 + MG_NCAND * (max_wi * p->nroot + 1) * 8 + g->max_tiles * 64 +
                          MG_TAP_FT * MG_TAP_KS * 64 * 8 + 512 + 2 * p->KK * 64 * 4 + 256;
        g->cs_ok = g->mfma_ok && g->max_tiles <= mg_cs_max_tiles(p->KK) && g->cs_lds_bytes <= budget1 && (int)g->chunks.size() <= MG_ARG_CHUNKS;
    }
}

static int mg_grid_build(mg_primitive *p, mg_time_grid *g, const double *times, int32_t T,
                         const int32_t *i0_override, const double *w_override) {
    g->prim = p;
    g->T = T;
    g->times.assign(times, times + T);
    g->i0.resize(T);
    g->w.resize((size_t)T * 4);
    for (int f = 0; f < T; f++) {
        if (i0_override) {
            g->i0[f] = i0_override[f];
            for (int j = 0; j < 4; j++) g->w[4 * f + j] = w_override[4 * f + j];
        } else {
            mg_basis_row(p->knots.data(), (int)p->knots.size(), times[f], &g->i0[f], &g->w[4 * f]);
        }
    }
    mg_plan_chunks(p, g);
    std::vector<float> w32(g->w.size());
    for (size_t q = 0; q < g->w.size(); q++) w32[q] = (float)g->w[q];
    MG_HIP_CHECK(hipSetDevice(p->ctx->device));
    int rc;
    if ((rc = mg_upload(p->ctx, g->i0, &g->d_i0)) != MG_OK) return rc;
    if ((rc = mg_upload(p->ctx, g->w, &g->d_w)) != MG_OK) return rc;
    if ((rc = mg_upload(p->ctx, w32, &g->d_w32)) != MG_OK) return rc;
    {
        std::vector<float> rootm((size_t)std::max(T, 1) * 8, 0.0f);
        for (int f = 0; f < T; f++)
            for (int d = 0; d < p->nroot; d++) {
                const double *m = &p->means_[(size_t)g->i0[f] * p->D + d];
                double M = g->w[4 * (size_t)f] * m[0];
                for (int j = 1; j < 4; j++) M = std::fma(g->w[4 * (size_t)f + j], m[(size_t)j * p->D], M);
                const float hi = (float)M;
                rootm[8 * (size_t)f + d] = hi;
                rootm[8 * (size_t)f + 3 + d] = (float)(M - (double)hi);
            }
        if ((rc = mg_upload(p->ctx, rootm, &g->d_rootm)) != MG_OK) return rc;
    }
    if ((rc = mg_upload(p->ctx, g->chunks, &g->d_chunks)) != MG_OK) return rc;
    {
        std::vector<double> wtap(std::max<size_t>(g->chunks.size(), 1) * MG_TAP_FT * MG_TAP_KS * 64, 0.0);
        for (size_t c = 0; c < g->chunks.size(); c++) {
            const mg_chunk &ck = g->chunks[c];
            for (int ft = 0; ft < MG_TAP_FT; ft++)
                for (int ks = 0; ks < MG_TAP_KS; ks++)
                    for (int lane = 0; lane < 64; lane++) {
                        int f = ft * 16 + (lane & 15), m = 4 * ks + (lane >> 4);
                        if (f >= ck.nT) continue;
                        int j = m - (g->i0[ck.t0 + f] - ck.imin);
                        if (j >= 0 && j < 4) wtap[((c * MG_TAP_FT + ft) * MG_TAP_KS + ks) * 64 + lane] = g->w[4 * (size_t)(ck.t0 + f) + j];
                    }
        }
        if ((rc = mg_upload(p->ctx, wtap, &g->d_wtap)) != MG_OK) return rc;
    }
    return MG_OK;
}

extern "C" int mg_time_grid_create(mg_primitive *prim, const double *times, int32_t n_times, mg_time_grid **out) {
    MG_REQUIRE(prim && out && n_times >= 0 && (n_times == 0 || times), "mg_time_grid_create: bad arguments");
    *out = nullptr;
    for (int i = 0; i < n_times; i++) MG_REQUIRE(std::isfinite(times[i]), "mg_time_grid_create: times[%d] is not finite", i);
    mg_time_grid *g = new (std::nothrow) mg_time_grid();
    if (!g) return MG_ERR_OUT_OF_MEMORY;
    int rc = mg_grid_build(prim, g, times, n_times, nullptr, nullptr);
    if (rc != MG_OK) { mg_free_grid_device(g); delete g; return rc; }
    *out = g;
    return MG_OK;
}
extern "C" void mg_time_grid_destroy(mg_time_grid *g) {
    if (!g || g->owned_by_prim) return;
    if (g->prim) (void)hipStreamSynchronize(g->prim->ctx->stream);
    mg_free_grid_device(g);
    delete g;
}
extern "C" mg_time_grid *mg_primitive_canonical_grid(mg_primitive *prim) { return prim ? prim->canonical : nullptr; }
extern "C" int mg_time_grid_size(const mg_time_grid *g) { return g ? g->T : 0; }
extern "C" int mg_time_grid_get_tables(const mg_time_grid *g, int32_t *i0, double *weights, double *times) {
    MG_REQUIRE(g != nullptr, "mg_time_grid_get_tables: grid is NULL");
    if (i0) std::copy(g->i0.begin(), g->i0.end(), i0);
    if (weights) std::copy(g->w.begin(), g->w.end(), weights);
    if (times) std::copy(g->times.begin(), g->times.end(), times);
    return MG_OK;
}

static void mg_primitive_free(mg_primitive *p) {
    if (!p) return;
    (void)hipSetDevice(p->ctx->device);
    (void)hipStreamSynchronize(p->ctx->stream);
    void *ptrs[] = {p->d_Epack, p->d_Et32, p->d_Et64, p->d_Erpack, p->d_meanroot, p->d_mean32, p->d_mean, p->d_knots,
                    p->d_gP, p->d_gmP, p->d_gconst, p->d_gmean, p->d_gchol, p->d_gPpack, p->d_gmPpad, p->d_gPTpack, p->d_gcholpack, p->d_gmeanpad,
                    p->d_tphi, p->d_tmean};
    for (void *q : ptrs) mg_dev_free(p->ctx, q);
    for (mg_time_grid *g : {p->canonical, p->coeff_grid})
        if (g) { mg_free_grid_device(g); delete g; }
    delete p;
}

extern "C" void mg_primitive_destroy(mg_primitive *p) {
    if (p && p->ctx) p->ctx->fused_next.valid = false;
    mg_primitive_free(p);
}

extern "C" int mg_primitive_create(mg_context *ctx, const mg_primitive_desc *d, mg_primitive **out) {
    MG_REQUIRE(ctx && d && out, "mg_primitive_create: NULL argument");
    *out = nullptr;
    MG_REQUIRE(d->n_basis >= 4, "mg_primitive_create: n_basis = %d, a cubic spline needs >= 4", d->n_basis);
    MG_REQUIRE(d->n_dim >= 1 && d->n_components >= 1 && d->n_canonical_frames >= 1,
               "mg_primitive_create: n_dim/n_components/n_canonical_frames must be >= 1");
    MG_REQUIRE(d->n_gmm >= 0, "mg_primitive_create: n_gmm < 0");
    MG_REQUIRE(d->eigen_vectors && d->mean_vector && d->knots, "mg_primitive_create: eigen_vectors/mean_vector/knots are required");
    MG_REQUIRE(d->n_gmm == 0 || (d->gmm_weights && d->gmm_means && d->gmm_covars),
               "mg_primitive_create: gmm arrays are required when n_gmm > 0");
    MG_REQUIRE((int64_t)d->n_basis * d->n_dim < (1 << 24), "mg_primitive_create: n_basis*n_dim too large");
    const int NB = d->n_basis, D = d->n_dim, L = d->n_components, K = d->n_gmm, R = NB * D;
    const int Lg = d->n_gmm_dims > 0 ? d->n_gmm_dims : L;
    MG_REQUIRE(Lg >= L, "mg_primitive_create: n_gmm_dims = %d < n_components = %d", Lg, L);
    const int Lt = d->n_time_components, NBt = d->n_basis_time;
    MG_REQUIRE(Lt >= 0 && (Lt == 0 || (NBt >= 4 && d->eigen_vectors_time && d->mean_time_vector && d->knots_time)),
               "mg_primitive_create: a time model needs n_basis_time >= 4, eigen_vectors_time, mean_time_vector and knots_time");
    for (int i = 0; i + 1 < NB + 4; i++)
        MG_REQUIRE(d->knots[i] <= d->knots[i + 1] && std::isfinite(d->knots[i + 1]), "mg_primitive_create: knots must be finite and non-decreasing");
    MG_REQUIRE(d->knots[3] < d->knots[NB], "mg_primitive_create: knot vector has an empty domain");
    MG_HIP_CHECK(hipSetDevice(ctx->device));

    mg_primitive *p = new (std::nothrow) mg_primitive();
    if (!p) return MG_ERR_OUT_OF_MEMORY;
    p->ctx = ctx;
    p->NB = NB; p->D = D; p->L = L; p->F = d->n_canonical_frames; p->K = K; p->R = R;
    p->nroot = std::min(3, D);
    p->KK = (L <= 4 * MG_MAX_KK) ? (((L + 3) / 4 + 1) / 2) * 2 : 0;
    p->Lg = Lg;
    p->KKg = (Lg <= 4 * MG_MAX_KK) ? (((Lg + 3) / 4 + 1) / 2) * 2 : 0;
    p->Lt = Lt; p->NBt = NBt;
    p->cshift = (4 - p->nroot) & 3;
    p->Dp = (D + p->cshift + 3) & ~3;
    p->RT = (NB * p->Dp + 15) / 16;
    p->knots.assign(d->knots, d->knots + NB + 4);
    double tm[3] = {1.0, 1.0, 1.0};
    if (d->translation_maxima)
        for (int i = 0; i < 3; i++) tm[i] = d->translation_maxima[i];

    p->Es.resize((size_t)R * L);
    p->means_.resize(R);
    for (int r = 0; r < R; r++) {
        double sc = (r % D < 3) ? tm[r % D] : 1.0;
        for (int k = 0; k < L; k++) {
            double e = d->eigen_is_transposed ? d->eigen_vectors[(size_t)r * L + k] : d->eigen_vectors[(size_t)k * R + r];
            p->Es[(size_t)r * L + k] = e * sc;
        }
        p->means_[r] = d->mean_vector[r] * sc;
    }

    int rc = MG_OK;
    {
        std::vector<float> et32((size_t)L * R);
        std::vector<double> et64((size_t)L * R);
        for (int r = 0; r < R; r++)
            for (int k = 0; k < L; k++) {
                et64[(size_t)k * R + r] = p->Es[(size_t)r * L + k];
                et32[(size_t)k * R + r] = (float)p->Es[(size_t)r * L + k];
            }
        if (rc == MG_OK) rc = mg_upload(ctx, et32, &p->d_Et32);
        if (rc == MG_OK) rc = mg_upload(ctx, et64, &p->d_Et64);
        if (rc == MG_OK) rc = mg_upload(ctx, p->means_, &p->d_mean);
        if (rc == MG_OK) rc = mg_upload(ctx, p->knots, &p->d_knots);
        {
            std::vector<float> m32((size_t)p->RT * 16, 0.0f);
            for (int i = 0; i < NB; i++)
                for (int dd = p->nroot; dd < D; dd++)
                    m32[(size_t)i * p->Dp + dd + p->cshift] = (float)p->means_[(size_t)i * D + dd];
            if (rc == MG_OK) rc = mg_upload(ctx, m32, &p->d_mean32);
        }
        if (rc == MG_OK && p->KK > 0) {
            const int KK = p->KK, nr = p->nroot, RR = NB * nr;
            p->RRT = (RR + 15) / 16;
            std::vector<double> rpack((size_t)p->RRT * KK * 64, 0.0), mroot((size_t)p->RRT * 16, 0.0);
            for (int rr = 0; rr < RR; rr++) mroot[rr] = p->means_[(size_t)(rr / nr) * D + rr % nr];
            for (int t = 0; t < p->RRT; t++)
                for (int kk = 0; kk < KK; kk++)
                    for (int lane = 0; lane < 64; lane++) {
                        int rr = t * 16 + (lane & 15), k = 4 * kk + (lane >> 4);
                        if (rr < RR && k < L)
                            rpack[((size_t)t * KK + kk) * 64 + lane] = p->Es[((size_t)(rr / nr) * D + rr % nr) * L + k];
                    }
            rc = mg_upload(ctx, rpack, &p->d_Erpack);
            if (rc == MG_OK) rc = mg_upload(ctx, mroot, &p->d_meanroot);
        }
        if (rc == MG_OK && p->KK > 0) {
            const int KK = p->KK, Dp = p->Dp;
            std::vector<float> pack((size_t)p->RT * KK * 64, 0.0f);
            for (int rt = 0; rt < p->RT; rt++)
                for (int kk = 0; kk < KK; kk++)
                    for (int lane = 0; lane < 64; lane++) {
                        int rp = rt * 16 + (lane & 15), k = 4 * kk + (lane >> 4);
                        int i = rp / Dp, dd = rp - i * Dp - p->cshift;
                        float v = (i < NB && dd >= 0 && dd < D && k < L) ? (float)p->Es[((size_t)i * D + dd) * L + k] : 0.0f;
                        pack[(((size_t)rt * (KK / 2) + kk / 2) * 64 + lane) * 2 + (kk & 1)] = v;
                    }
            {
                const size_t n1 = pack.size();
                pack.resize(2 * n1, 0.0f);
                for (int rt = 0; rt < p->RT; rt++)
                    for (int kk = 0; kk < KK; kk++)
                        for (int lane = 0; lane < 64; lane++) {
                            const float v = pack[(((size_t)rt * (KK / 2) + kk / 2) * 64 + lane) * 2 + (kk & 1)];
                            const int q = kk / 4, nq = KK / 4;
                            const size_t tile = n1 + (size_t)rt * KK * 64;
                            if (q < nq) pack[tile + ((size_t)q * 64 + lane) * 4 + (kk & 3)] = v;
                            else pack[tile + (size_t)nq * 256 + (size_t)lane * 2 + (kk & 1)] = v;
                        }
            }
            rc = mg_upload(ctx, pack, &p->d_Epack);
        }
    }
    if (rc != MG_OK) { mg_primitive_free(p); return rc; }

    if (K > 0) {
        p->gw.assign(d->gmm_weights, d->gmm_weights + K);
        p->gm.assign(d->gmm_means, d->gmm_means + (size_t)K * Lg);
        p->gc.assign(d->gmm_covars, d->gmm_covars + (size_t)K * Lg * Lg);
        p->gp.assign((size_t)K * Lg * Lg, 0.0);
        std::vector<double> chol((size_t)K * Lg * Lg), inv((size_t)Lg * Lg);
        std::vector<double> gP((size_t)K * Lg * Lg, 0.0), gmP((size_t)K * Lg), gconst(K);
        const double log2pi = std::log(2.0 * M_PI);
        for (int k = 0; k < K; k++) {
            double *c = &chol[(size_t)k * Lg * Lg];
            if (!(p->gw[k] >= 0.0) || !std::isfinite(p->gw[k])) {
                mg_set_error("mg_primitive_create: gmm_weights[%d] is negative or not finite", k);
                mg_primitive_free(p);
                return MG_ERR_INVALID_ARGUMENT;
            }
            if (!mg_cholesky_lower(&p->gc[(size_t)k * Lg * Lg], Lg, c)) {
                mg_set_error("mg_primitive_create: gmm_covars[%d] is not positive definite", k);
                mg_primitive_free(p);
                return MG_ERR_NOT_POSITIVE_DEFINITE;
            }
            std::fill(inv.begin(), inv.end(), 0.0);
            for (int col = 0; col < Lg; col++)
                for (int r = col; r < Lg; r++) {
                    double s = (r == col) ? 1.0 : 0.0;
                    for (int q = col; q < r; q++) s -= c[r * Lg + q] * inv[(size_t)q * Lg + col];
                    inv[(size_t)r * Lg + col] = s / c[r * Lg + r];
                }
            double *P = &p->gp[(size_t)k * Lg * Lg];
            double logdet = 0.0;
            for (int i = 0; i < Lg; i++) {
                for (int j = 0; j < Lg; j++) P[i * Lg + j] = inv[(size_t)j * Lg + i];
// ... 932 lines not shown
}
extern "C" int mg_back_project_frames_f64_host(mg_primitive *p, const mg_time_grid *g, const void *lat, int dt,
                                               int64_t B, int64_t ld, double *frames) {
    int rc = mg_check_latents("mg_back_project_frames_f64_host", p, lat, dt, B, ld);
    if (rc != MG_OK) return rc;
    if (!g) g = p->canonical;
    int64_t ob = B * (int64_t)g->T * p->D * 8;
    mg_host_io io;
    if ((rc = io.stage(p->ctx, lat, B * ld * (int64_t)mg_dt_size(dt), ob)) != MG_OK) return rc;
    if ((rc = mg_back_project_frames_f64(p, g, io.d_in, dt, B, ld, (double *)io.d_out)) != MG_OK) return rc;
    return io.finish(frames, ob);
}
extern "C" int mg_back_project_coeffs_host(mg_primitive *p, const void *lat, int dt, int64_t B, int64_t ld,
                                           void *coeffs, int odt) {
    int rc = mg_check_latents("mg_back_project_coeffs_host", p, lat, dt, B, ld);
    if (rc != MG_OK) return rc;
    MG_REQUIRE(odt == MG_F32 || odt == MG_F64, "mg_back_project_coeffs_host: bad output dtype %d", odt);
    int64_t ob = B * (int64_t)p->R * (int64_t)mg_dt_size(odt);
    mg_host_io io;
    if ((rc = io.stage(p->ctx, lat, B * ld * (int64_t)mg_dt_size(dt), ob)) != MG_OK) return rc;
    if ((rc = mg_back_project_coeffs(p, io.d_in, dt, B, ld, io.d_out, odt)) != MG_OK) return rc;
    return io.finish(coeffs, ob);
}
extern "C" int mg_spline_evaluate_host(mg_primitive *p, const mg_time_grid *g, const double *coeffs, int64_t n, double *frames) {
    MG_REQUIRE(p != nullptr && n >= 0, "mg_spline_evaluate_host: bad arguments");
    if (!g) g = p->canonical;
    int64_t ib = n * (int64_t)p->R * 8, ob = n * (int64_t)g->T * p->D * 8;
    mg_host_io io;
    int rc;
    if ((rc = io.stage(p->ctx, coeffs, ib, ob)) != MG_OK) return rc;
    if ((rc = mg_spline_evaluate(p, g, (const double *)io.d_in, n, (double *)io.d_out)) != MG_OK) return rc;
    return io.finish(frames, ob);
}
extern "C" int mg_time_function_canonical_host(mg_primitive *p, const void *gamma, int gdt, int64_t B, int64_t ld, double *out) {
    MG_REQUIRE(p != nullptr && B >= 0 && (gdt == MG_F32 || gdt == MG_F64), "mg_time_function_canonical_host: bad arguments");
    int64_t ob = B * (int64_t)p->F * 8;
    mg_host_io io;
    int rc;
    if ((rc = io.stage(p->ctx, gamma, B * ld * (int64_t)mg_dt_size(gdt), ob)) != MG_OK) return rc;
    if ((rc = mg_time_function_canonical(p, io.d_in, gdt, B, ld, (double *)io.d_out)) != MG_OK) return rc;
    return io.finish(out, ob);
}
extern "C" int mg_gmm_log_prob_host(mg_primitive *p, const void *x, int xdt, int64_t B, int64_t ld, void *logp, int odt) {
    int rc = mg_check_mixture_rows("mg_gmm_log_prob_host", p, x, xdt, B, ld);
    if (rc != MG_OK) return rc;
    MG_REQUIRE(odt == MG_F32 || odt == MG_F64, "mg_gmm_log_prob_host: bad output dtype %d", odt);
    int64_t ob = B * (int64_t)mg_dt_size(odt);
    mg_host_io io;
    if ((rc = io.stage(p->ctx, x, B * ld * (int64_t)mg_dt_size(xdt), ob)) != MG_OK) return rc;
    if ((rc = mg_gmm_log_prob(p, io.d_in, xdt, B, ld, io.d_out, odt)) != MG_OK) return rc;
    return io.finish(logp, ob);
}
extern "C" int mg_gmm_sample_host(mg_primitive *p, int64_t n, const int64_t *counts, uint64_t seed, void *x, int xdt,
                                  int64_t ld, int32_t *comp) {
    MG_REQUIRE(p != nullptr && n >= 0 && ld >= (p ? p->Lg : 0), "mg_gmm_sample_host: bad arguments");
    MG_REQUIRE(xdt == MG_F32 || xdt == MG_F64, "mg_gmm_sample_host: bad dtype %d", xdt);
    int64_t xb = n * ld * (int64_t)mg_dt_size(xdt), cb = n * 4;
    void *dx = nullptr, *dc = nullptr;
    int rc = mg_device_malloc(p->ctx, xb, &dx);
    if (rc != MG_OK) return rc;
    rc = mg_device_malloc(p->ctx, cb, &dc);
    if (rc == MG_OK) rc = mg_memset(p->ctx, dx, 0, xb);
    if (rc == MG_OK) rc = mg_gmm_sample(p, n, counts, seed, dx, xdt, ld, (int32_t *)dc);
    if (rc == MG_OK) rc = mg_memcpy_d2h(p->ctx, x, dx, xb);
    if (rc == MG_OK && comp) rc = mg_memcpy_d2h(p->ctx, comp, dc, cb);
    (void)mg_device_free(p->ctx, dx);
    (void)mg_device_free(p->ctx, dc);
    return rc;
}
extern "C" int mg_score_constraint_residuals_host(mg_primitive *p, const mg_constraint_set *cs, const void *lat, int dt,
                                                  int64_t B, int64_t ld, double *res) {
    int rc = mg_check_latents("mg_score_constraint_residuals_host", p, lat, dt, B, ld);
    if (rc != MG_OK) return rc;
    MG_REQUIRE(cs && cs->prim == p, "mg_score_constraint_residuals_host: constraint set is NULL or belongs to another primitive");
    int64_t ob = B * (int64_t)cs->n * 8;
    mg_host_io io;
    if ((rc = io.stage(p->ctx, lat, B * ld * (int64_t)mg_dt_size(dt), ob)) != MG_OK) return rc;
    if ((rc = mg_score_constraint_residuals(p, cs, io.d_in, dt, B, ld, (double *)io.d_out)) != MG_OK) return rc;
    return io.finish(res, ob);
}
extern "C" int mg_gmm_log_prob_jac_host(mg_primitive *p, const void *x, int xdt, int64_t B, int64_t ld, double *jac) {
    int rc = mg_check_mixture_rows("mg_gmm_log_prob_jac_host", p, x, xdt, B, ld);
    if (rc != MG_OK) return rc;
    int64_t ob = B * (int64_t)p->Lg * 8;
    mg_host_io io;
    if ((rc = io.stage(p->ctx, x, B * ld * (int64_t)mg_dt_size(xdt), ob)) != MG_OK) return rc;
    if ((rc = mg_gmm_log_prob_jac(p, io.d_in, xdt, B, ld, (double *)io.d_out)) != MG_OK) return rc;
    return io.finish(jac, ob);
}
extern "C" int mg_score_constraints_host(mg_primitive *p, const mg_constraint_set *cs, const void *lat, int dt,
                                         int64_t B, int64_t ld, void *errors, int odt) {
    int rc = mg_check_latents("mg_score_constraints_host", p, lat, dt, B, ld);
    if (rc != MG_OK) return rc;
    MG_REQUIRE(odt == MG_F32 || odt == MG_F64, "mg_score_constraints_host: bad output dtype %d", odt);
    int64_t ob = B * (int64_t)mg_dt_size(odt);
    mg_host_io io;
    if ((rc = io.stage(p->ctx, lat, B * ld * (int64_t)mg_dt_size(dt), ob)) != MG_OK) return rc;
    if ((rc = mg_score_constraints(p, cs, io.d_in, dt, B, ld, io.d_out, odt)) != MG_OK) return rc;
    return io.finish(errors, ob);
}

static int mg_best_candidate_impl(const char *who, mg_primitive *p, const mg_constraint_set *cs, const void *lat_dev, int dt,
                                  int64_t B, int64_t ld, void *err_dev, int64_t *best, double *minv) {
    MG_REQUIRE(cs && cs->prim == p, "%s: constraint set is NULL or belongs to another primitive", who);
    if (B == 0) {
        if (best) *best = 0;
        if (minv) *minv = INFINITY;
        return MG_OK;
    }
    int rc = mg_score_constraints(p, cs, lat_dev, dt, B, ld, err_dev, MG_F64);
    if (rc != MG_OK) return rc;
    return mg_argmin_first(p->ctx, err_dev, MG_F64, B, best, minv);
}
extern "C" int mg_best_candidate(mg_primitive *p, const mg_constraint_set *cs, const void *lat, int dt, int64_t B,
                                 int64_t ld, int64_t *best, double *minv) {
    int rc = mg_check_latents("mg_best_candidate", p, lat, dt, B, ld);
    if (rc != MG_OK) return rc;
    void *err = nullptr;
    if ((rc = mg_ctx_scratch(p->ctx, std::max<int64_t>(B, 1) * 8, &err)) != MG_OK) return rc;
    return mg_best_candidate_impl("mg_best_candidate", p, cs, lat, dt, B, ld, err, best, minv);
}
extern "C" int mg_best_candidate_host(mg_primitive *p, const mg_constraint_set *cs, const void *lat, int dt, int64_t B,
                                      int64_t ld, int64_t *best, double *minv) {
    int rc = mg_check_latents("mg_best_candidate_host", p, lat, dt, B, ld);
    if (rc != MG_OK) return rc;
    mg_host_io io;
    if ((rc = io.stage(p->ctx, lat, B * ld * (int64_t)mg_dt_size(dt), std::max<int64_t>(B, 1) * 8)) != MG_OK) return rc;
    return mg_best_candidate_impl("mg_best_candidate_host", p, cs, io.d_in, dt, B, ld, io.d_out, best, minv);
}

extern "C" int mg_option_step_rows(mg_primitive *p, const mg_constraint_set *cs, int64_t n, const int64_t *counts, uint64_t seed,
                                   int64_t row_begin, int64_t row_count, void *x_dev, int xdt, int64_t ld, double *errors_dev, void *result_dev) {
    MG_REQUIRE(p && cs && cs->prim == p, "mg_option_step: constraint set is NULL or belongs to another primitive");
    MG_REQUIRE(n > 0 && row_count > 0 && x_dev && errors_dev && result_dev, "mg_option_step: bad arguments");
    int rc = mg_gmm_sample_rows(p, n, counts, seed, row_begin, row_count, x_dev, xdt, ld, nullptr);
    if (rc == MG_OK) rc = mg_score_constraints(p, cs, x_dev, xdt, row_count, ld, errors_dev, MG_F64);
    if (rc == MG_OK) {
        mg_prof_begin(p->ctx, 3);
        rc = mg_launch_argmin_gather(p->ctx, errors_dev, MG_F64, row_count, result_dev, x_dev, xdt, ld, p->Lg, row_begin);
        mg_prof_end(p->ctx, 3);
    }
    return rc;
}
extern "C" int mg_option_step(mg_primitive *p, const mg_constraint_set *cs, int64_t n, const int64_t *counts, uint64_t seed,
                              void *x_dev, int xdt, int64_t ld, double *errors_dev, void *result_dev) {
    return mg_option_step_rows(p, cs, n, counts, seed, 0, n, x_dev, xdt, ld, errors_dev, result_dev);
}

static int mg_ctx_pinned(mg_context *ctx, size_t bytes) {
    if (ctx->pinned_bytes < bytes) {
        MG_HIP_CHECK(hipStreamSynchronize(ctx->stream));
        if (ctx->pinned) (void)hipHostFree(ctx->pinned);
        ctx->pinned = nullptr; ctx->pinned_bytes = 0;
        const size_t cap = std::max<size_t>(bytes, 64 * 1024);
        MG_HIP_CHECK(hipHostMalloc(&ctx->pinned, cap, hipHostMallocDefault));
        memset(ctx->pinned, 0, cap);
        ctx->pinned_bytes = cap;
    }
    return MG_OK;
}
static int mg_ctx_flags(mg_context *ctx, size_t n, unsigned long long **out) {
    if (ctx->flag_cap < n) {
        MG_HIP_CHECK(hipStreamSynchronize(ctx->stream));
        if (ctx->flag_block) (void)hipHostFree(ctx->flag_block);
        ctx->flag_block = nullptr; ctx->flag_cap = 0;
        const size_t cap = std::max<size_t>(n, 64);
        MG_HIP_CHECK(hipHostMalloc((void **)&ctx->flag_block, cap * sizeof(unsigned long long), hipHostMallocDefault));
        ctx->flag_cap = cap;
    }
    for (size_t k = 0; k < n; k++) ((volatile unsigned long long *)ctx->flag_block)[k] = 0ull;
    __atomic_thread_fence(__ATOMIC_RELEASE);
    *out = ctx->flag_block;
    return MG_OK;
}
static int mg_wait_flags(mg_context *ctx, const volatile unsigned long long *flags, int n, unsigned long long seq) {
    struct timespec t0 = {0, 0};
    bool have_t0 = false, synced = false;
    for (int k = 0; k < n; k++) {
        unsigned spins = 0;
        while (flags[k] != seq && !synced) {
            __builtin_ia32_pause();
            if ((++spins & 1023u) != 0) continue;
            struct timespec t1;
            clock_gettime(CLOCK_MONOTONIC, &t1);
            if (!have_t0) { t0 = t1; have_t0 = true; continue; }
            if ((t1.tv_sec - t0.tv_sec) * 1000000000L + (t1.tv_nsec - t0.tv_nsec) > 2000000L) {
                MG_HIP_CHECK(hipStreamSynchronize(ctx->stream));
                synced = true;
            }
        }
        if (flags[k] != seq) { mg_set_error("mg_options_step: the step's kernel finished without writing its result records"); return MG_ERR_HIP; }
    }
    __atomic_thread_fence(__ATOMIC_ACQUIRE);
    return MG_OK;
}
static int mg_read_back_pinned(mg_context *ctx, void *dst, const void *src_dev, size_t bytes) {
    { int rcp = mg_ctx_pinned(ctx, bytes); if (rcp != MG_OK) return rcp; }
    MG_HIP_CHECK(hipMemcpyAsync(ctx->pinned, src_dev, bytes, hipMemcpyDeviceToHost, ctx->stream));
    MG_HIP_CHECK(hipStreamSynchronize(ctx->stream));
    memcpy(dst, ctx->pinned, bytes);
    return MG_OK;
}

static int mg_ctx_side_streams(mg_context *ctx) {
    if (ctx->side[0]) return MG_OK;
    for (auto &st : ctx->side) MG_HIP_CHECK(hipStreamCreateWithFlags(&st, hipStreamNonBlocking));
    for (auto &e : ctx->side_ev) MG_HIP_CHECK(hipEventCreateWithFlags(&e, hipEventDisableTiming));
    return MG_OK;
}

extern "C" int mg_options_step(int32_t n_options, mg_primitive *const *prims, const mg_constraint_set *const *csets, int64_t n,
                               const int64_t *const *counts, const uint64_t *seeds, void *const *x_dev, int xdt, const int64_t *ld,
                               double *const *errors_dev, void *results_dev, int64_t result_stride, void *results_host) {
    return mg_options_step_rows(n_options, prims, csets, n, counts, seeds, 0, n, x_dev, xdt, ld, errors_dev, results_dev, result_stride, results_host);
}
extern "C" int mg_options_step_device_counts(int32_t n_options, mg_primitive *const *prims, const mg_constraint_set *const *csets, int64_t n,
                                             const uint64_t *seeds, void *const *x_dev, int xdt, const int64_t *ld,
                                             double *const *errors_dev, void *results_dev, int64_t result_stride, void *results_host,
                                             int64_t *counts_host) {
    MG_REQUIRE(n_options > 0 && n_options <= 24 && prims && csets && seeds && x_dev && ld && errors_dev && results_dev && n > 0,
               "mg_options_step_device_counts: bad arguments (at most 24 options)");
    mg_context *ctx = prims[0] ? prims[0]->ctx : nullptr;
    for (int k = 0; k < n_options; k++) {
        MG_REQUIRE(prims[k] && prims[k]->ctx == ctx, "mg_options_step_device_counts: option %d is NULL or lives in another context", k);
        MG_REQUIRE(result_stride >= 16 + 8 * (int64_t)prims[k]->Lg && result_stride % 8 == 0, "mg_options_step_device_counts: result_stride %lld too small for option %d",
                   (long long)result_stride, k);
        MG_REQUIRE(csets[k] && csets[k]->prim == prims[k], "mg_options_step_device_counts: constraint set %d is NULL or belongs to another primitive", k);
        MG_REQUIRE(x_dev[k] && errors_dev[k] && ld[k] >= prims[k]->Lg, "mg_options_step_device_counts: bad arguments for option %d", k);
    }
    MG_REQUIRE(xdt == MG_F32 || xdt == MG_F64, "mg_options_step_device_counts: bad dtype %d", xdt);
    { int rc0 = mg_use_device(ctx); if (rc0 != MG_OK) return rc0; }
    if (!mg_options_can_fuse(n_options, prims, csets, n)) {
        mg_set_error("mg_options_step_device_counts: an option does not run on the one-launch kernel (mixture of more than 16 components or 64 dimensions, "
                     "constraint tables beyond LDS, or a VALU kernel forced): draw the counts on the host and call mg_options_step");
        return MG_ERR_UNSUPPORTED;
    }
    const size_t rec_bytes = ((size_t)n_options * (size_t)result_stride + 63) / 64 * 64,
                 cnt_bytes = (size_t)n_options * MG_SAMPLE_ARG_K * sizeof(int32_t);
    char *rec_host = nullptr;
    int32_t *cnt_host = nullptr;
    unsigned long long *flags = nullptr;
    if (results_host || counts_host) {
        int rcp = mg_ctx_pinned(ctx, rec_bytes + cnt_bytes);
        if (rcp != MG_OK) return rcp;
        rec_host = (char *)ctx->pinned;
        rcp = mg_ctx_flags(ctx, (size_t)n_options, &flags);
        if (rcp != MG_OK) return rcp;
        if (counts_host) cnt_host = (int32_t *)(rec_host + rec_bytes);
    }
    const unsigned long long seq = ++ctx->fused_seq;
    int rc = mg_launch_options_fused(n_options, prims, csets, n, nullptr, seeds, x_dev, xdt, ld, errors_dev, results_dev, result_stride, 0, n, rec_host, cnt_host,
                                     flags, seq);
    if (rc != MG_OK) return rc;
    if (results_host || counts_host) {
        int rcw = mg_wait_flags(ctx, flags, n_options, seq);
        if (rcw != MG_OK) return rcw;
        if (results_host) memcpy(results_host, rec_host, (size_t)n_options * (size_t)result_stride);
        if (counts_host)
            for (size_t i = 0; i < (size_t)n_options * MG_SAMPLE_ARG_K; i++) counts_host[i] = cnt_host[i];
    }
    return MG_OK;
}

extern "C" int mg_options_step_rows(int32_t n_options, mg_primitive *const *prims, const mg_constraint_set *const *csets, int64_t n,
                                    const int64_t *const *counts, const uint64_t *seeds, int64_t row_begin, int64_t row_count,
                                    void *const *x_dev, int xdt, const int64_t *ld,
                                    double *const *errors_dev, void *results_dev, int64_t result_stride, void *results_host) {
    MG_REQUIRE(n_options > 0 && prims && csets && counts && seeds && x_dev && ld && errors_dev && results_dev, "mg_options_step: bad arguments");
    MG_REQUIRE(row_begin >= 0 && row_count > 0 && row_begin + row_count <= n, "mg_options_step_rows: rows [%lld, %lld) outside the draw of %lld",
               (long long)row_begin, (long long)(row_begin + row_count), (long long)n);
    mg_context *ctx = prims[0] ? prims[0]->ctx : nullptr;
    for (int k = 0; k < n_options; k++) {
        MG_REQUIRE(prims[k] && prims[k]->ctx == ctx, "mg_options_step: option %d is NULL or lives in another context", k);
        MG_REQUIRE(result_stride >= 16 + 8 * (int64_t)prims[k]->Lg && result_stride % 8 == 0, "mg_options_step: result_stride %lld too small for option %d",
                   (long long)result_stride, k);
    }
    { int rc0 = mg_use_device(ctx); if (rc0 != MG_OK) return rc0; }
    for (int k = 0; k < n_options; k++) {
        MG_REQUIRE(csets[k] && csets[k]->prim == prims[k], "mg_options_step: constraint set %d is NULL or belongs to another primitive", k);
        MG_REQUIRE(n > 0 && counts[k] && x_dev[k] && errors_dev[k] && ld[k] >= prims[k]->Lg, "mg_options_step: bad arguments for option %d", k);
    }
    MG_REQUIRE(xdt == MG_F32 || xdt == MG_F64, "mg_options_step: bad dtype %d", xdt);
    {
        bool fused = true;
        for (int k0 = 0; k0 < n_options && fused; k0 += 24) fused = mg_options_can_fuse(std::min(24, n_options - k0), prims + k0, csets + k0, n);
        if (fused) {
            char *rec_host = nullptr;
            unsigned long long *flags = nullptr;
            const size_t rec_bytes = ((size_t)n_options * (size_t)result_stride + 63) / 64 * 64;
            if (results_host) {
                int rcp = mg_ctx_pinned(ctx, rec_bytes);
                if (rcp != MG_OK) return rcp;
                rec_host = (char *)ctx->pinned;
                rcp = mg_ctx_flags(ctx, (size_t)n_options, &flags);
                if (rcp != MG_OK) return rcp;
            }
            const unsigned long long seq = ++ctx->fused_seq;
            for (int k0 = 0; k0 < n_options; k0 += 24) {
                int rcf = mg_launch_options_fused(std::min(24, n_options - k0), prims + k0, csets + k0, n, counts + k0, seeds + k0, x_dev + k0, xdt, ld + k0,
                                                  errors_dev + k0, (char *)results_dev + (size_t)k0 * result_stride, result_stride, row_begin, row_count,
                                                  rec_host ? rec_host + (size_t)k0 * result_stride : nullptr, nullptr, flags ? flags + k0 : nullptr, seq);
                if (rcf != MG_OK) return rcf;
            }
            if (results_host) {
                int rcw = mg_wait_flags(ctx, flags, n_options, seq);
                if (rcw != MG_OK) return rcw;
                memcpy(results_host, rec_host, (size_t)n_options * (size_t)result_stride);
            }
            return MG_OK;
        }
    }
    bool shared_scratch = false;
    for (int k = 0; k < n_options; k++) shared_scratch = shared_scratch || !mg_gmm_sample_takes_host_prefix(prims[k]);
    const int S = (n_options >= 4 && !shared_scratch) ? 4 : 1;
    if (S > 1) {
        int rcs = mg_ctx_side_streams(ctx);
        if (rcs != MG_OK) return rcs;
    }
    hipStream_t main_stream = ctx->stream;
    if (S > 1) {
        MG_HIP_CHECK(hipEventRecord(ctx->side_ev[4], main_stream));
        for (int i = 0; i < S; i++) MG_HIP_CHECK(hipStreamWaitEvent(ctx->side[i], ctx->side_ev[4], 0));
    }
    int rc = MG_OK;
    for (int k = 0; k < n_options && rc == MG_OK; k++) {
        if (S > 1) ctx->stream = ctx->side[k % S];
        rc = mg_option_step_rows(prims[k], csets[k], n, counts[k], seeds[k], row_begin, row_count, x_dev[k], xdt, ld[k], errors_dev[k],
                                 (char *)results_dev + k * result_stride);
    }
    ctx->stream = main_stream;
    if (S > 1) {
        for (int i = 0; i < S; i++) {
            (void)hipEventRecord(ctx->side_ev[i], ctx->side[i]);
            (void)hipStreamWaitEvent(main_stream, ctx->side_ev[i], 0);
        }
    }
    if (rc != MG_OK) return rc;
    if (results_host) return mg_read_back_pinned(ctx, results_host, results_dev, (size_t)(n_options * result_stride));
    return MG_OK;
}
```

### morphablegraphs_amd/csrc/mg_internal.h

```cpp
#pragma once
#include <hip/hip_runtime.h>

#include <cstdint>
#include <map>
#include <string>
#include <vector>

#include "../../include/mg_hip.h"

#define MG_NCAND 16
#define MG_ROWTILE 16
#define MG_MAX_KK 16
#define MG_BLOCK 256
#define MG_PROFILE_SLOTS 15

void mg_set_error(const char *fmt, ...);
int mg_hip_fail(hipError_t e, const char *what);

#define MG_HIP_CHECK(expr)                                   \
    do {                                                     \
        hipError_t _e = (expr);                              \
        if (_e != hipSuccess) return mg_hip_fail(_e, #expr); \
    } while (0)

#define MG_REQUIRE_AS(cond, code, ...) \
    do {                               \
        if (!(cond)) {                 \
            mg_set_error(__VA_ARGS__); \
            return (code);             \
        }                              \
    } while (0)

struct mg_event_pair {
    hipEvent_t a, b;
    int slot;
    bool ended;
    int slot2 = -1;
};

struct mg_context {
    int device = 0;
    hipStream_t stream = nullptr;
    bool own_stream = false;
    int n_cu = 0;
    int64_t total_mem = 0;
    int max_lds = 0;
    char name[256] = {0};
    bool profile = false;
    std::vector<mg_event_pair> pending;
    std::vector<hipEvent_t> free_events;
    int reserved_cus = 0;
    int32_t opt[MG_OPT_COUNT] = {0};
    int prof_interval = 1;
    int64_t prof_seen[MG_PROFILE_SLOTS] = {0};
    double prof_ms[MG_PROFILE_SLOTS] = {0};
    int64_t prof_n[MG_PROFILE_SLOTS] = {0};
    std::vector<float> prof_samples[MG_PROFILE_SLOTS];
    void *scratch = nullptr;
    int64_t scratch_bytes = 0;
    void *argmin_out = nullptr;
    struct arena_block { char *base; size_t bytes, used; int64_t live; };
    std::vector<arena_block> arena;
    size_t arena_block_bytes = 0;
    struct vmm_alloc { void *va; size_t total, chunk; std::vector<hipMemGenericAllocationHandle_t> handles; };
    std::vector<vmm_alloc> vmm;
    std::vector<std::pair<void *, size_t>> vmm_parked;
    hipStream_t side[4] = {nullptr, nullptr, nullptr, nullptr};
    hipEvent_t side_ev[5] = {nullptr, nullptr, nullptr, nullptr, nullptr};
    void *fused_tab_dev = nullptr;
    std::vector<unsigned char> fused_tab_host;
    void *fused_counters = nullptr, *fused_partials = nullptr;
    void *fused_dyn_dev = nullptr;
    struct { bool valid = false; int32_t n_options = 0, slot = 0; int64_t n = 0; uint64_t seeds[24] = {0}; const void *prims[24] = {nullptr}; } fused_next;
    unsigned attr_gmm_lds = 0, attr_traj = 0;
    unsigned long long fused_seq = 0;
    int fused_partials_n = 0;
    struct out_region {
        char *base = nullptr; size_t bytes = 0; bool vmm = false, fast = false; double ratio = 1.0, us = 0.0, tbps = 0.0; int probed = 0;
        std::vector<std::pair<size_t, size_t>> free_list;
        std::map<size_t, size_t> used;
        int64_t live = 0;
    };
    std::vector<out_region> out_regions;
    void *pinned = nullptr;
    size_t pinned_bytes = 0;
    unsigned long long *flag_block = nullptr;
    size_t flag_cap = 0;
    void *traj_paths = nullptr;
    size_t traj_paths_bytes = 0;
    void *lists_dev = nullptr;
    size_t lists_bytes = 0, lists_counters_off = 0;
    void *rccl_comm = nullptr;
    int dist_rank = 0, dist_ranks = 1;
    void *tree_tab_dev = nullptr;
    size_t tree_tab_cap = 0;
    std::vector<unsigned char> tree_tab_host;
    void *walk_tab_dev = nullptr;
    size_t walk_tab_cap = 0;
    std::vector<unsigned char> walk_tab_host;
    void *wscore_tab_dev = nullptr;
    size_t wscore_tab_cap = 0;
    std::vector<unsigned char> wscore_tab_host;
    void *wtime_tab_dev = nullptr;
    size_t wtime_tab_cap = 0;
    std::vector<unsigned char> wtime_tab_host;
    int64_t wtime_tab_uploads = 0;
    void *slen_tab_dev = nullptr;
    size_t slen_tab_cap = 0;
    std::vector<unsigned char> slen_tab_host;
};
void mg_dev_free(mg_context *ctx, void *p);

int mg_ctx_scratch(mg_context *ctx, int64_t bytes, void **out);
void mg_prof_begin(mg_context *ctx, int slot);
bool mg_prof_kernel(mg_context *ctx, int slot, int slot2, hipEvent_t *start, hipEvent_t *stop);
void mg_prof_end(mg_context *ctx, int slot);
int mg_prof_resolve(mg_context *ctx);

#define MG_MAX_WI 11
#define MG_MAX_NT 48
#define MG_TAP_KS ((MG_MAX_WI + 3) / 4)
#define MG_TAP_FT (MG_MAX_NT / 16)
#define MG_ARG_CHUNKS 8
#define MG_RO_PAD 8
#define MG_RO_CS(nt) ((nt) * 4 + MG_RO_PAD)
#define MG_TB_BYTES_N(nt) ((nt) * 16 + (nt) * 4)
#define MG_RO_BYTES_N(nt) (MG_NCAND * MG_RO_CS(nt) * 4)
struct mg_chunk {
    int32_t t0;
    int32_t nT;
    int32_t rt0;
    int32_t ntiles;
    int32_t imin;
    int32_t wi;
    int32_t rrt0;
    int32_t nrt;
};

struct mg_time_grid {
    mg_primitive *prim = nullptr;
    bool owned_by_prim = false;
    int32_t T = 0;
    std::vector<double> times;
    std::vector<int32_t> i0;
    std::vector<double> w;
    std::vector<mg_chunk> chunks;
    int32_t *d_i0 = nullptr;
    double *d_w = nullptr;
    float *d_w32 = nullptr;
    float *d_rootm = nullptr;
    double *d_wtap = nullptr;
    mg_chunk *d_chunks = nullptr;
    int32_t n_chunks = 0;
    int32_t stride = 0;
    int32_t max_wi = 0;
    int32_t max_nt = 16;
    int32_t lds_bytes = 0;
    int32_t nbuf = 2;
    bool mfma_ok = false;
    int32_t max_tiles = 0;
    int32_t cs_lds_bytes = 0;
    bool cs_ok = false;
};

struct mg_primitive {
    mg_context *ctx = nullptr;
    int32_t NB = 0, D = 0, L = 0, F = 0, K = 0, R = 0;
    int32_t nroot = 0;
    bool root_split = false;
    double root_split_est = 0.0;
    int32_t KK = 0;
    int32_t Lg = 0;
    int32_t KKg = 0;
    int32_t Lt = 0, NBt = 0;
    double *d_tphi = nullptr;
    double *d_tmean = nullptr;
    int32_t RT = 0;
    std::vector<double> Es;
    std::vector<double> means_;
    std::vector<double> knots;
    std::vector<double> gw, gm, gc, gp;
    int32_t Dp = 0;
    int32_t cshift = 0;
    float *d_Epack = nullptr;
    float *d_Et32 = nullptr;
    double *d_Et64 = nullptr;
    double *d_Erpack = nullptr;
    double *d_meanroot = nullptr;
    float *d_mean32 = nullptr;
    double *d_mean = nullptr;
    double *d_knots = nullptr;
    int32_t RRT = 0;
    double *d_gPpack = nullptr;
    double *d_gmPpad = nullptr;
    double *d_gP = nullptr;
    double *d_gmP = nullptr;
    double *d_gPTpack = nullptr;
    double *d_gcholpack = nullptr;
    double *d_gmeanpad = nullptr;
    double *d_gconst = nullptr;
    double *d_gmean = nullptr;
    double *d_gchol = nullptr;
    mg_time_grid *canonical = nullptr;
    mg_time_grid *coeff_grid = nullptr;
};

struct mg_constraint_set {
    mg_primitive *prim = nullptr;
    int32_t n = 0;
    int32_t nch = 0;
    double *d_W = nullptr;
    double *d_bias = nullptr;
    double *d_par = nullptr;
    int32_t *d_woff = nullptr;
    int32_t *d_chain = nullptr;
    double *d_choff = nullptr;
    double *d_Wpack = nullptr;
    double *d_bpad = nullptr;
    int32_t RT = 0;
    int32_t rows = 0;
    std::vector<mg_keyframe_constraint> structure;
    int32_t align_joint = -1;
    double *d_pose = nullptr;
    bool has_pose = false;
    double *d_align = nullptr;
};

struct mg_score_args {
    const double *W;
    const double *bias;
    const double *par;
    const int32_t *woff;
    const int32_t *chain;
    const double *choff;
    const double *pose;
    const double *align;
    const double *align_cand;
    const void *lat;
    void *out;
    double *res;
    int64_t B, ld;
    int32_t n, nch, L;
};

inline mg_score_args mg_score_args_of(const mg_constraint_set *cs, int32_t L) {
    mg_score_args a = {};
    a.W = cs->d_W; a.bias = cs->d_bias; a.par = cs->d_par; a.woff = cs->d_woff; a.chain = cs->d_chain; a.choff = cs->d_choff;
    a.pose = cs->d_pose; a.align = cs->d_align;
    a.n = cs->n; a.nch = cs->nch; a.L = L;
    return a;
}

#define MG_POSE_HDR 8
#define MG_POSE_REC (5 + 4 * MG_MAX_CHAIN)

int mg_launch_frames_mfma(mg_primitive *p, const mg_time_grid *g, const void *lat, int ldt, int64_t B, int64_t ld, float *out, float *logp,
                          int prof_slot = -1, int prof_slot2 = -1);
bool mg_frames_can_fuse_gmm(const mg_primitive *p, const mg_time_grid *g, int64_t B);
int mg_frames_kernel_choice(const mg_primitive *p, const mg_time_grid *g, int64_t B, bool fused, const void *out = nullptr, bool lat_f64 = false);
int mg_output_class(mg_context *ctx, const void *p);
int mg_frames_lds_bytes(const mg_primitive *p, const mg_time_grid *g, int which, bool fused);
int mg_frames_grid(const mg_primitive *p, const mg_time_grid *g, int64_t B, int which);
bool mg_frames_root_split(const mg_primitive *p);
#define MG_ROOT_SPLIT_MAX_EST 5e-6
int mg_cs_max_tiles(int KK);
int mg_launch_frames_direct(mg_primitive *p, const mg_time_grid *g, const void *lat, int ldt, int64_t B, int64_t ld, void *out, bool out_f64);
int mg_launch_spline_eval(mg_primitive *p, const mg_time_grid *g, const double *coeffs, int64_t n, double *out);
int mg_launch_gmm_logp(mg_primitive *p, const void *x, int xdt, int64_t B, int64_t ld, void *out, int odt);
bool mg_objective_can_fuse(const mg_primitive *p, const mg_constraint_set *cs);
int mg_launch_objective(mg_primitive *p, const mg_constraint_set *cs, const void *x, int xdt, int64_t B, int64_t ld, double error_scale,
                        double quality_scale, double *logp_out, double *err_out, double *obj_out);
#define MG_SAMPLE_ARG_K 16
int mg_launch_gmm_sample(mg_primitive *p, int64_t n, const int64_t *cum_dev, const int64_t *cum_host, int64_t n_tiles, uint64_t seed, void *x, int xdt, int64_t ld, int32_t *comp,
                         int64_t tile0, int64_t row_lo, int64_t row_hi);
bool mg_gmm_sample_takes_host_prefix(const mg_primitive *p);
int mg_launch_set_params(mg_context *ctx, const double *values, int n_par, int n_align, double *d_par, double *d_align);
int mg_launch_score(mg_primitive *p, const mg_constraint_set *cs, const void *lat, int ldt, int64_t B, int64_t ld, void *out, int odt, double *res,
                    const double *align_cand = nullptr);
int mg_launch_gather_winner(mg_context *ctx, const void *x, int xdt, int64_t ld, int L, void *result_dev);
int mg_launch_argmin_gather(mg_context *ctx, const void *v, int dt, int64_t n, void *result_dev, const void *x, int xdt, int64_t ld, int L, int64_t index_offset = 0);
int mg_launch_gmm_jac(mg_primitive *p, const void *x, int xdt, int64_t B, int64_t ld, double *out);
int mg_launch_time_function(mg_primitive *p, const void *gamma, int gdt, int64_t B, int64_t ld, double *out);
int mg_launch_timewarp(mg_primitive *p, const void *gamma, int gdt, int64_t B, int64_t ld, double speed, double *times, int32_t *lens, int32_t t_cap,
                       int64_t row_pitch, double *canonical_out);
int mg_launch_frames_at(mg_primitive *p, const void *lat, int ldt, int64_t B, int64_t ld, const double *times, const int32_t *lens, int32_t t_cap,
                        void *out, int odt);
int mg_launch_argmin(mg_context *ctx, const void *v, int dt, int64_t n, void *out_dev);
int mg_launch_joint_positions(mg_context *ctx, const double *frames, const double *table, int64_t N, int D, int J, double *out);
int mg_setup_kernel_attributes(mg_context *ctx);
int mg_options_fused_attributes();
bool mg_options_can_fuse(int32_t n_options, mg_primitive *const *prims, const mg_constraint_set *const *csets, int64_t n);
int mg_launch_options_fused(int32_t n_options, mg_primitive *const *prims, const mg_constraint_set *const *csets, int64_t n,
                            const int64_t *const *counts, const uint64_t *seeds, void *const *x_dev, int xdt, const int64_t *ld,
                            double *const *errors_dev, void *results_dev, int64_t result_stride, int64_t row_begin, int64_t row_count,
                            void *records_host = nullptr, int32_t *counts_host = nullptr, unsigned long long *flags_host = nullptr,
                            unsigned long long seq = 0);
int mg_probe_placement(mg_context *ctx, void *buf, int64_t bytes, double *ratio, double *pattern_us);
#define MG_PLACED_MIN_BYTES ((int64_t)64 << 20)
int mg_output_alloc(mg_context *ctx, int64_t bytes, int32_t max_candidates, void **out, double *info4);
bool mg_output_free(mg_context *ctx, void *p);
void mg_output_release_all(mg_context *ctx);
int mg_device_free_raw(mg_context *ctx, void *p);

void mg_basis_row(const double *knots, int n_knots, double x, int32_t *i0, double *w4);

struct mg_trajectory {
    mg_primitive *prim = nullptr;
    int32_t n_seg = 0, granularity = 1000, rows = 0;
    double *d_poly = nullptr;
    double *d_arc = nullptr;
    double full_arc = 0.0;
    double *d_E = nullptr;
    double *d_mean = nullptr;
};
```

### morphablegraphs_amd/csrc/mg_placement.hip

```cpp
#include <algorithm>
#include <map>
#include <vector>
#include <hip/hip_ext.h>

#include "mg_internal.h"

typedef float f32x4p __attribute__((ext_vector_type(4)));
typedef f32x4p f32x4pu __attribute__((aligned(4)));

#define MG_PP_T 156
#define MG_PP_D 79
#define MG_PP_NF 39
#define MG_PP_NCH 4
__global__ __launch_bounds__(512) void mg_placement_pattern_kernel(float *out, int ntiles) {
    const int wave = threadIdx.x >> 6, lane = threadIdx.x & 63;
    const int fsub = lane / 20, ql = lane % 20;
    const bool on = lane < 60;
    const int U = ntiles * MG_PP_NCH, per = (U + (int)gridDim.x - 1) / (int)gridDim.x;
    for (int s = 0; s < per; s++) {
        const int u = blockIdx.x * per + s;
        if (u >= U) break;
        const int tile = u / MG_PP_NCH, chunk = (u % MG_PP_NCH + blockIdx.x) % MG_PP_NCH;
        for (int f0 = 0; f0 < MG_PP_NF; f0 += 3)
            for (int half = 0; half < 2; half++) {
// ... 47 lines not shown
    float ms_fill = 0.f, ms_pat = 0.f;
    for (int i = 0; i < reps && e == hipSuccess; i++) {
        float ms = 0.f;
        e = hipEventElapsedTime(&ms, ev[2 * i], ev[2 * i + 1]);
        ms_fill += ms;
        if (e == hipSuccess) { e = hipEventElapsedTime(&ms, ev[2 * reps + 2 * i], ev[2 * reps + 2 * i + 1]); ms_pat += ms; }
    }
    if (e == hipSuccess) e = hipGetLastError();
    for (auto &x : ev) (void)hipEventDestroy(x);
    if (e != hipSuccess) return mg_hip_fail(e, "mg_probe_placement");
    *ratio = ms_fill > 0.f ? (double)ms_pat / (double)ms_fill : 1.0;
    *pattern_us = 1e3 * (double)ms_pat / reps;
    return MG_OK;
}

extern "C" int mg_device_probe_placement(mg_context *ctx, void *buf, int64_t bytes, double *info) {
    if (!ctx || !buf || !info || bytes < MG_PLACED_MIN_BYTES) {
        mg_set_error("mg_device_probe_placement: needs a context, a buffer of at least 64 MiB and info4");
        return MG_ERR_INVALID_ARGUMENT;
    }
    MG_HIP_CHECK(hipSetDevice(ctx->device));
    double ratio = 1.0, us = 0.0;
    int rc = mg_probe_placement(ctx, buf, bytes, &ratio, &us);
    if (rc != MG_OK) return rc;
    info[0] = 1.0; info[1] = ratio; info[2] = us; info[3] = mg_placement_is_fast(bytes, ratio, us, MG_PLACED_FAST_RATIO, MG_PLACED_CLASS_TBPS) ? 1.0 : 0.0;
    return MG_OK;
}

extern "C" int mg_device_placement_info(mg_context *ctx, const void *buf, double *info, double *tbps) {
    if (!ctx || !buf || !info) { mg_set_error("mg_device_placement_info: needs a context, a pointer and info4"); return MG_ERR_INVALID_ARGUMENT; }
    info[0] = 0.0; info[1] = 1.0; info[2] = 0.0; info[3] = 0.0;
    if (tbps) *tbps = 0.0;
    for (const auto &r : ctx->out_regions)
        if (r.base && (const char *)buf >= r.base && (const char *)buf < r.base + r.bytes) {
            info[0] = 1.0; info[1] = r.ratio; info[2] = r.us; info[3] = r.fast ? 1.0 : 0.0;
            if (tbps) *tbps = r.tbps;
            return MG_OK;
        }
    return MG_OK;
}

#define MG_REGION_GRANULE ((size_t)2 << 20)

static void mg_region_release(mg_context *ctx, mg_context::out_region &r) {
    if (!r.base) return;
    if (r.vmm) (void)mg_device_free_raw(ctx, r.base); else (void)hipFree(r.base);
    r.base = nullptr;
}

static int mg_region_create(mg_context *ctx, size_t bytes, size_t probe_bytes, int32_t max_candidates, mg_context::out_region *out) {
    size_t free_b = 0, total_b = 0;
    MG_HIP_CHECK(hipMemGetInfo(&free_b, &total_b));
    const int budget = max_candidates > 0 ? max_candidates : 32;
    size_t hold_cap = std::max<size_t>(free_b / 4, 2 * bytes);
    if (ctx->opt[MG_OPT_PLACED_HOLD] > 0) hold_cap = std::max<size_t>((size_t)ctx->opt[MG_OPT_PLACED_HOLD], 2) * bytes;
    const double fast_ratio = ctx->opt[MG_OPT_PLACED_FAST_PCT] > 0 ? ctx->opt[MG_OPT_PLACED_FAST_PCT] / 100.0 : MG_PLACED_FAST_RATIO;
    struct cand { void *p; bool vmm; };
    std::vector<cand> held;
    cand best = {nullptr, false};
    double best_ratio = 0.0, best_us = 0.0;
    bool best_fast = false;
    int probed = 0, rc = MG_OK;
    auto drop = [&](const cand &c) { if (c.vmm) (void)mg_device_free_raw(ctx, c.p); else (void)hipFree(c.p); };
    auto consider = [&](void *p, bool vmm) -> bool {
        double ratio = 1.0, us = 0.0;
        rc = mg_probe_placement(ctx, p, (int64_t)probe_bytes, &ratio, &us);
        if (rc != MG_OK) { drop({p, vmm}); return false; }
        probed++;
        if (!best.p || (us > 0.0 && best_us > 0.0 ? us < best_us : ratio < best_ratio)) {
            if (best.p) held.push_back(best);
            best = {p, vmm}; best_ratio = ratio; best_us = us;
            best_fast = mg_placement_is_fast((int64_t)probe_bytes, ratio, us, fast_ratio);
        } else {
            held.push_back({p, vmm});
        }
        while (!held.empty() && (held.size() + 2) * bytes > hold_cap) {
            (void)hipStreamSynchronize(ctx->stream);
            drop(held.front());
            held.erase(held.begin());
        }
        return !best_fast;
    };
    int limit = budget;
    auto plain = [&](int count) {
        for (int i = 0; i < count && probed < limit; i++) {
            void *p = nullptr;
            if (hipMalloc(&p, bytes) != hipSuccess) { (void)hipGetLastError(); return; }
            if (!consider(p, false)) return;
        }
    };
    plain(std::min(budget, 16));
    if (best.p && !best_fast && rc == MG_OK && max_candidates != 1) {
        static const int64_t chunk_mib[3] = {32, 8, 2};
        bool go = true;
        for (int c = 0; c < 3 && go; c++)
            for (int i = 0; i < 4 && go && probed < budget; i++) {
                void *p = nullptr;
                if (mg_device_malloc_chunked(ctx, (int64_t)bytes, chunk_mib[c] << 20, &p) != MG_OK) { (void)hipGetLastError(); go = false; break; }
                go = consider(p, true);
            }
        if (rc == MG_OK && !best_fast) plain(budget - probed);
    }
    if (rc == MG_OK && best.p && !best_fast && max_candidates == 0 && ctx->opt[MG_OPT_PLACED_HOLD] == 0) {
        limit = MG_PLACED_DEEP_CANDIDATES;
        hold_cap = std::max<size_t>(hold_cap, free_b / 10 * 6);
        while (probed < limit && !best_fast && rc == MG_OK && (held.size() + 3) * bytes <= hold_cap) {
            const int before = probed;
            plain(1);
            if (probed == before) break;
        }
    }
    (void)hipStreamSynchronize(ctx->stream);
    for (const cand &c : held) drop(c);
    if (rc != MG_OK) {
        if (best.p) drop(best);
        return rc;
    }
    if (!best.p) {
        mg_set_error("mg_device_malloc: out of device memory (%lld bytes)", (long long)bytes);
        return MG_ERR_OUT_OF_MEMORY;
    }
    out->base = (char *)best.p; out->bytes = bytes; out->vmm = best.vmm; out->ratio = best_ratio; out->us = best_us;
    out->tbps = mg_placement_tbps((int64_t)probe_bytes, best_us);
    out->probed = probed; out->fast = best_fast || mg_placement_is_fast((int64_t)probe_bytes, best_ratio, best_us, fast_ratio, MG_PLACED_CLASS_TBPS);
    out->live = 0;
    out->free_list.clear();
    out->free_list.push_back({0, bytes});
    return MG_OK;
}

int mg_output_alloc(mg_context *ctx, int64_t bytes, int32_t max_candidates, void **out, double *info) {
    const size_t need = ((size_t)bytes + MG_REGION_GRANULE - 1) / MG_REGION_GRANULE * MG_REGION_GRANULE;
    for (int pass = 0; pass < 2; pass++) {
        for (auto &r : ctx->out_regions) {
            if (pass == 0 && !r.fast) continue;
            for (size_t i = 0; i < r.free_list.size(); i++) {
                if (r.free_list[i].second < need) continue;
                *out = r.base + r.free_list[i].first;
                r.used[(char *)*out - r.base] = need;
                if (r.free_list[i].second == need) r.free_list.erase(r.free_list.begin() + (long)i);
                else { r.free_list[i].first += need; r.free_list[i].second -= need; }
                r.live++;
                if (info) { info[0] = 0.0; info[1] = r.ratio; info[2] = r.us; info[3] = r.fast ? 1.0 : 0.0; }
                return MG_OK;
            }
        }
    }
    bool released = false;
    for (size_t i = ctx->out_regions.size(); i-- > 0;)
        if (ctx->out_regions[i].live == 0) {
            if (!released) { (void)hipStreamSynchronize(ctx->stream); released = true; }
            mg_region_release(ctx, ctx->out_regions[i]);
            ctx->out_regions.erase(ctx->out_regions.begin() + (long)i);
        }
    mg_context::out_region r;
    int rc = mg_region_create(ctx, need, (size_t)bytes, max_candidates, &r);
    if (rc == MG_ERR_OUT_OF_MEMORY) {
        void *p = nullptr;
        if (hipMalloc(&p, need) != hipSuccess) {
            (void)hipGetLastError();
            mg_set_error("mg_device_malloc: out of device memory (%lld bytes)", (long long)need);
            return MG_ERR_OUT_OF_MEMORY;
        }
        r = mg_context::out_region();
        r.base = (char *)p; r.bytes = need; r.vmm = false; r.fast = false; r.ratio = 1.0; r.us = 0.0; r.probed = 0;
        rc = MG_OK;
    }
    if (rc != MG_OK) return rc;
    *out = r.base;
    r.used[0] = need;
    r.free_list.clear();
    r.live = 1;
    if (info) { info[0] = r.probed; info[1] = r.ratio; info[2] = r.us; info[3] = r.fast ? 1.0 : 0.0; }
    ctx->out_regions.push_back(std::move(r));
    return MG_OK;
}

bool mg_output_free(mg_context *ctx, void *p) {
    for (auto &r : ctx->out_regions) {
        if ((char *)p < r.base || (char *)p >= r.base + r.bytes) continue;
        const size_t off = (size_t)((char *)p - r.base);
        auto it = r.used.find(off);
        if (it == r.used.end()) return false;
        std::pair<size_t, size_t> blk = {off, it->second};
        r.used.erase(it);
        r.live--;
        size_t i = 0;
        while (i < r.free_list.size() && r.free_list[i].first < blk.first) i++;
        r.free_list.insert(r.free_list.begin() + (long)i, blk);
        if (i + 1 < r.free_list.size() && r.free_list[i].first + r.free_list[i].second == r.free_list[i + 1].first) {
            r.free_list[i].second += r.free_list[i + 1].second;
            r.free_list.erase(r.free_list.begin() + (long)i + 1);
        }
        if (i > 0 && r.free_list[i - 1].first + r.free_list[i - 1].second == r.free_list[i].first) {
            r.free_list[i - 1].second += r.free_list[i].second;
            r.free_list.erase(r.free_list.begin() + (long)i);
        }
        return true;
    }
    return false;
}

void mg_output_release_all(mg_context *ctx) {
    for (auto &r : ctx->out_regions) mg_region_release(ctx, r);
    ctx->out_regions.clear();
}

extern "C" int mg_context_trim_outputs(mg_context *ctx) {
    if (!ctx) { mg_set_error("mg_context_trim_outputs: ctx is NULL"); return MG_ERR_INVALID_ARGUMENT; }
    MG_HIP_CHECK(hipSetDevice(ctx->device));
    MG_HIP_CHECK(hipStreamSynchronize(ctx->stream));
    for (size_t i = ctx->out_regions.size(); i-- > 0;)
        if (ctx->out_regions[i].live == 0) {
            mg_region_release(ctx, ctx->out_regions[i]);
            ctx->out_regions.erase(ctx->out_regions.begin() + (long)i);
        }
    return MG_OK;
}

int mg_output_class(mg_context *ctx, const void *p) {
    if (!ctx || !p) return -1;
    for (const auto &r : ctx->out_regions)
        if (r.base && (const char *)p >= r.base && (const char *)p < r.base + r.bytes) return r.fast ? 1 : 0;
    return -1;
}

extern "C" int mg_context_output_bytes(mg_context *ctx, int64_t *reserved, int64_t *in_use, int32_t *n_regions, int32_t *n_fast) {
    if (!ctx) { mg_set_error("mg_context_output_bytes: ctx is NULL"); return MG_ERR_INVALID_ARGUMENT; }
    int64_t res = 0, use = 0;
    int32_t nf = 0;
    for (auto &r : ctx->out_regions) {
        res += (int64_t)r.bytes;
        for (auto &u : r.used) use += (int64_t)u.second;
        nf += r.fast ? 1 : 0;
    }
    if (reserved) *reserved = res;
    if (in_use) *in_use = use;
    if (n_regions) *n_regions = (int32_t)ctx->out_regions.size();
    if (n_fast) *n_fast = nf;
    return MG_OK;
}

extern "C" int mg_device_malloc_placed(mg_context *ctx, int64_t bytes, int32_t max_candidates, void **out_dev, double *info) {
    if (!ctx || !out_dev || bytes < 0) {
        mg_set_error("mg_device_malloc_placed: bad arguments");
        return MG_ERR_INVALID_ARGUMENT;
    }
    *out_dev = nullptr;
    MG_HIP_CHECK(hipSetDevice(ctx->device));
    if (info) { info[0] = 0.0; info[1] = 1.0; info[2] = 0.0; info[3] = 1.0; }
    if (bytes < MG_PLACED_MIN_BYTES) return mg_device_malloc(ctx, bytes, out_dev);
    return mg_output_alloc(ctx, bytes, max_candidates, out_dev, info);
}
```

Before: 109.9 million samples/s.

## Cache frames launch plans and spin-poll stream completion instead of blocking sync

Adds a per-primitive cache of the planned launch arguments, LDS size, grid and resolved kernel-instance function pointer. A generation counter bumped on option, CU-reservation and output-region changes invalidates it, so repeated steps skip the planning logic. Replaces blocking hipStreamSynchronize with a bounded busy-poll on hipStreamQuery before falling back to a blocking sync, and routes small device-to-host copies through the pinned staging buffer. The aim is to cut per-call host overhead and wake-up latency, at the cost of CPU spinning and stale-cache risk if some invalidation path is missed.

```diff
diff --git a/morphablegraphs_amd/csrc/mg_frames.hip b/morphablegraphs_amd/csrc/mg_frames.hip
--- a/morphablegraphs_amd/csrc/mg_frames.hip
+++ b/morphablegraphs_amd/csrc/mg_frames.hip
@@ -1,4 +1,5 @@
 #include "mg_frames_common.h"
+#include <new>
 
 int mg_setup_kernel_attributes(mg_context *) {
     int rc = mg_frames_ws_attributes();
@@ -52,9 +53,26 @@
     return g->lds_bytes + (fused ? mg_fused_gmm_lds(p) : 0);
 }
 
-int mg_launch_frames_mfma(mg_primitive *p, const mg_time_grid *g, const void *lat, int ldt, int64_t B, int64_t ld, float *out, float *logp,
-                          int prof_slot, int prof_slot2) {
+struct mg_step_cache {
+    bool valid = false;
+    uint64_t gen = 0;
+    const mg_time_grid *g = nullptr;
+    int64_t B = 0, ld = 0;
+    int ldt = 0;
+    bool fused = false;
+    const void *out = nullptr;
+    int out_class = -1;
     mg_frames_args a;
+    int buf_bytes = 0, lds = 0, grid = 0;
+    mg_frames_launch_fn fn = nullptr;
+};
+void mg_frames_cache_drop(mg_primitive *p) {
+    delete p->step_cache;
+    p->step_cache = nullptr;
+}
+
+static int mg_frames_plan_launch(mg_primitive *p, const mg_time_grid *g, int ldt, int64_t B, int64_t ld, const void *out, bool fused, mg_step_cache *r) {
+    mg_frames_args &a = r->a;
     a.rt_total = p->RT;
     a.B = B; a.ld = ld; a.T = g->T; a.D = p->D; a.Dp = p->Dp; a.cshift = p->cshift; a.L = p->L; a.nroot = p->nroot;
     a.n_chunks = g->n_chunks; a.stride = g->stride; a.max_wi = g->max_wi; a.max_nt = g->max_nt; a.nbuf = g->nbuf;
@@ -69,7 +87,7 @@
     for (int i = 0; i < MG_ARG_CHUNKS; i++) a.ck[i] = i < g->n_chunks ? g->chunks[i] : mg_chunk{};
     a.cs_magic = a.cs_per = a.cs_rem = 0;
     const bool lf = (ldt == MG_F64);
-    const int which = mg_frames_kernel_choice(p, g, B, logp != nullptr, out, lf);
+    const int which = mg_frames_kernel_choice(p, g, B, fused, out, lf);
     if (which < 0) {
         mg_set_error("mg_back_project_frames: the chunk-stationary kernel does not cover this shape (window of %d row tiles, %d bytes of LDS)",
                      g->max_tiles, g->cs_lds_bytes);
@@ -78,13 +96,13 @@
     const bool cs = which == 2;
     const int buf_bytes = (MG_NCAND * g->stride * 4 + 255) / 256 * 256;
     int lds = g->nbuf * (buf_bytes + MG_RO_BYTES_N(g->max_nt) + MG_TB_BYTES_N(g->max_nt)) + MG_NCAND * (g->max_wi * p->nroot + 1) * 8 + 128;
-    if (lds != g->lds_bytes || lds > 160 * 1024 || (logp && !mg_frames_can_fuse_gmm(p, g, B))) {
+    if (lds != g->lds_bytes || lds > 160 * 1024 || (fused && !mg_frames_can_fuse_gmm(p, g, B))) {
         mg_set_error("mg_back_project_frames: internal LDS sizing mismatch (%d vs %d)", lds, g->lds_bytes);
         return MG_ERR_UNSUPPORTED;
     }
     if (cs) lds = g->cs_lds_bytes;
-    a.gmm_staged = cs && logp && mg_fused_gmm_staged(p, g) ? 1 : 0;
-    if (logp) lds += a.gmm_staged ? mg_fused_gmm_lds_cs(p) : mg_fused_gmm_lds(p);
+    a.gmm_staged = cs && fused && mg_fused_gmm_staged(p, g) ? 1 : 0;
+    if (fused) lds += a.gmm_staged ? mg_fused_gmm_lds_cs(p) : mg_fused_gmm_lds(p);
     const int grid = mg_frames_grid(p, g, B, which);
     if (cs) {
         const int Q = grid / g->n_chunks;
@@ -92,9 +110,37 @@
         a.cs_per = (int32_t)(n_tiles / Q);
         a.cs_rem = (int32_t)(n_tiles % Q);
     }
+    const bool split = mg_frames_root_split(p);
+    r->fn = cs ? mg_frames_cs_instance(p, fused, lf, split) : mg_frames_ws_instance(p, fused, lf, split);
+    if (!r->fn) return MG_ERR_UNSUPPORTED;
+    r->gen = p->ctx->launch_gen;
+    r->g = g; r->B = B; r->ld = ld; r->ldt = ldt; r->fused = fused;
+    r->out = out; r->out_class = mg_output_class(p->ctx, out);
+    r->buf_bytes = buf_bytes; r->lds = lds; r->grid = grid;
+    return MG_OK;
+}
+
+int mg_launch_frames_mfma(mg_primitive *p, const mg_time_grid *g, const void *lat, int ldt, int64_t B, int64_t ld, float *out, float *logp,
+                          int prof_slot, int prof_slot2) {
+    mg_context *ctx = p->ctx;
+    const bool fused = logp != nullptr;
+    mg_step_cache *c = p->step_cache;
+    bool hit = c && c->valid && c->gen == ctx->launch_gen && c->g == g && c->B == B && c->ld == ld && c->ldt == ldt && c->fused == fused;
+    if (hit && out != c->out) {
+        hit = mg_output_class(ctx, out) == c->out_class;
+        if (hit) c->out = out;
+    }
+    mg_step_cache fresh;
+    if (!hit) {
+        const int rc = mg_frames_plan_launch(p, g, ldt, B, ld, out, fused, &fresh);
+        if (rc != MG_OK) return rc;
+        c = &fresh;
+        if (g->owned_by_prim) {
+            if (!p->step_cache) p->step_cache = new (std::nothrow) mg_step_cache();
+            if (p->step_cache) { *p->step_cache = fresh; p->step_cache->valid = true; c = p->step_cache; }
+        }
+    }
     mg_launch_events ev;
-    if (prof_slot >= 0) (void)mg_prof_kernel(p->ctx, prof_slot, prof_slot2, &ev.start, &ev.stop);
-    const bool split = mg_frames_root_split(p);
-    return cs ? mg_launch_frames_cs(p, g, lat, out, logp, a, lf, split, buf_bytes, lds, grid, ev)
-              : mg_launch_frames_ws(p, g, lat, out, logp, a, lf, split, buf_bytes, lds, grid, ev);
+    if (prof_slot >= 0) (void)mg_prof_kernel(ctx, prof_slot, prof_slot2, &ev.start, &ev.stop);
+    return c->fn(p, g, lat, out, logp, c->a, c->buf_bytes, c->lds, c->grid, ev);
 }
diff --git a/morphablegraphs_amd/csrc/mg_frames_common.h b/morphablegraphs_amd/csrc/mg_frames_common.h
--- a/morphablegraphs_amd/csrc/mg_frames_common.h
+++ b/morphablegraphs_amd/csrc/mg_frames_common.h
@@ -329,9 +329,9 @@
 
 
 struct mg_launch_events { hipEvent_t start = nullptr, stop = nullptr; };
-int mg_launch_frames_ws(mg_primitive *p, const mg_time_grid *g, const void *lat, float *out, float *logp, const mg_frames_args &a, bool lat_f64,
-                        bool split, int buf_bytes, int lds, int grid, const mg_launch_events &ev);
-int mg_launch_frames_cs(mg_primitive *p, const mg_time_grid *g, const void *lat, float *out, float *logp, const mg_frames_args &a, bool lat_f64,
-                        bool split, int buf_bytes, int lds, int grid, const mg_launch_events &ev);
+typedef int (*mg_frames_launch_fn)(mg_primitive *p, const mg_time_grid *g, const void *lat, float *out, float *logp, const mg_frames_args &a,
+                                   int buf_bytes, int lds, int grid, const mg_launch_events &ev);
+mg_frames_launch_fn mg_frames_ws_instance(const mg_primitive *p, bool fuse, bool lat_f64, bool split);
+mg_frames_launch_fn mg_frames_cs_instance(const mg_primitive *p, bool fuse, bool lat_f64, bool split);
 int mg_frames_ws_attributes();
 int mg_frames_cs_attributes();
diff --git a/morphablegraphs_amd/csrc/mg_frames_cs.hip b/morphablegraphs_amd/csrc/mg_frames_cs.hip
--- a/morphablegraphs_amd/csrc/mg_frames_cs.hip
+++ b/morphablegraphs_amd/csrc/mg_frames_cs.hip
@@ -663,39 +663,33 @@
 }
 
 template <int KK>
-static int mg_launch_cs_kk(mg_primitive *p, const mg_time_grid *g, const void *lat, float *out, float *logp, const mg_frames_args &a,
-                               bool lat_f64, bool split, int buf_bytes, int lds, int grid, const mg_launch_events &ev) {
-    if (logp) {
+static mg_frames_launch_fn mg_cs_inst_kk(bool fuse, bool lat_f64, bool split) {
+    if (fuse) {
         if constexpr (KK <= MG_FUSE_MAX_KK) {
-            if (split)
-                return lat_f64 ? mg_launch_cs_inst<KK, true, true, true>(p, g, lat, out, logp, a, buf_bytes, lds, grid, ev)
-                               : mg_launch_cs_inst<KK, false, true, true>(p, g, lat, out, logp, a, buf_bytes, lds, grid, ev);
-            return lat_f64 ? mg_launch_cs_inst<KK, true, true, false>(p, g, lat, out, logp, a, buf_bytes, lds, grid, ev)
-                           : mg_launch_cs_inst<KK, false, true, false>(p, g, lat, out, logp, a, buf_bytes, lds, grid, ev);
-        }
-        mg_set_error("mg_step_frames_and_logp: no fused kernel for %d components", p->L);
-        return MG_ERR_UNSUPPORTED;
-    }
-    if (split)
-        return lat_f64 ? mg_launch_cs_inst<KK, true, false, true>(p, g, lat, out, nullptr, a, buf_bytes, lds, grid, ev)
-                       : mg_launch_cs_inst<KK, false, false, true>(p, g, lat, out, nullptr, a, buf_bytes, lds, grid, ev);
-    return lat_f64 ? mg_launch_cs_inst<KK, true, false, false>(p, g, lat, out, nullptr, a, buf_bytes, lds, grid, ev)
-                   : mg_launch_cs_inst<KK, false, false, false>(p, g, lat, out, nullptr, a, buf_bytes, lds, grid, ev);
-}
-
-int mg_launch_frames_cs(mg_primitive *p, const mg_time_grid *g, const void *lat, float *out, float *logp, const mg_frames_args &a, bool lat_f64,
-                        bool split, int buf_bytes, int lds, int grid, const mg_launch_events &ev) {
+            if (split) return lat_f64 ? mg_launch_cs_inst<KK, true, true, true> : mg_launch_cs_inst<KK, false, true, true>;
+            return lat_f64 ? mg_launch_cs_inst<KK, true, true, false> : mg_launch_cs_inst<KK, false, true, false>;
+        }
+        return nullptr;
+    }
+    if (split) return lat_f64 ? mg_launch_cs_inst<KK, true, false, true> : mg_launch_cs_inst<KK, false, false, true>;
+    return lat_f64 ? mg_launch_cs_inst<KK, true, false, false> : mg_launch_cs_inst<KK, false, false, false>;
+}
+
+mg_frames_launch_fn mg_frames_cs_instance(const mg_primitive *p, bool fuse, bool lat_f64, bool split) {
+    mg_frames_launch_fn fn = nullptr;
     switch (p->KK) {
-        case 2: return mg_launch_cs_kk<2>(p, g, lat, out, logp, a, lat_f64, split, buf_bytes, lds, grid, ev);
-        case 4: return mg_launch_cs_kk<4>(p, g, lat, out, logp, a, lat_f64, split, buf_bytes, lds, grid, ev);
-        case 6: return mg_launch_cs_kk<6>(p, g, lat, out, logp, a, lat_f64, split, buf_bytes, lds, grid, ev);
-        case 8: return mg_launch_cs_kk<8>(p, g, lat, out, logp, a, lat_f64, split, buf_bytes, lds, grid, ev);
-        case 10: return mg_launch_cs_kk<10>(p, g, lat, out, logp, a, lat_f64, split, buf_bytes, lds, grid, ev);
-        case 12: return mg_launch_cs_kk<12>(p, g, lat, out, logp, a, lat_f64, split, buf_bytes, lds, grid, ev);
-        case 14: return mg_launch_cs_kk<14>(p, g, lat, out, logp, a, lat_f64, split, buf_bytes, lds, grid, ev);
-        case 16: return mg_launch_cs_kk<16>(p, g, lat, out, logp, a, lat_f64, split, buf_bytes, lds, grid, ev);
-        default: mg_set_error("mg_back_project_frames: MFMA path needs n_components <= 64"); return MG_ERR_UNSUPPORTED;
-    }
+        case 2: fn = mg_cs_inst_kk<2>(fuse, lat_f64, split); break;
+        case 4: fn = mg_cs_inst_kk<4>(fuse, lat_f64, split); break;
+        case 6: fn = mg_cs_inst_kk<6>(fuse, lat_f64, split); break;
+        case 8: fn = mg_cs_inst_kk<8>(fuse, lat_f64, split); break;
+        case 10: fn = mg_cs_inst_kk<10>(fuse, lat_f64, split); break;
+        case 12: fn = mg_cs_inst_kk<12>(fuse, lat_f64, split); break;
+        case 14: fn = mg_cs_inst_kk<14>(fuse, lat_f64, split); break;
+        case 16: fn = mg_cs_inst_kk<16>(fuse, lat_f64, split); break;
+        default: mg_set_error("mg_back_project_frames: MFMA path needs n_components <= 64"); return nullptr;
+    }
+    if (!fn) mg_set_error("mg_step_frames_and_logp: no fused kernel for %d components", p->L);
+    return fn;
 }
 
 template <int KK>
diff --git a/morphablegraphs_amd/csrc/mg_frames_ws.hip b/morphablegraphs_amd/csrc/mg_frames_ws.hip
--- a/morphablegraphs_amd/csrc/mg_frames_ws.hip
+++ b/morphablegraphs_amd/csrc/mg_frames_ws.hip
@@ -394,39 +394,33 @@
 }
 
 template <int KK>
-static int mg_launch_ws_kk(mg_primitive *p, const mg_time_grid *g, const void *lat, float *out, float *logp, const mg_frames_args &a,
-                               bool lat_f64, bool split, int buf_bytes, int lds, int grid, const mg_launch_events &ev) {
-    if (logp) {
+static mg_frames_launch_fn mg_ws_inst_kk(bool fuse, bool lat_f64, bool split) {
+    if (fuse) {
         if constexpr (KK <= MG_FUSE_MAX_KK) {
-            if (split)
-                return lat_f64 ? mg_launch_ws_inst<KK, true, true, true>(p, g, lat, out, logp, a, buf_bytes, lds, grid, ev)
-                               : mg_launch_ws_inst<KK, false, true, true>(p, g, lat, out, logp, a, buf_bytes, lds, grid, ev);
-            return lat_f64 ? mg_launch_ws_inst<KK, true, true, false>(p, g, lat, out, logp, a, buf_bytes, lds, grid, ev)
-                           : mg_launch_ws_inst<KK, false, true, false>(p, g, lat, out, logp, a, buf_bytes, lds, grid, ev);
-        }
-        mg_set_error("mg_step_frames_and_logp: no fused kernel for %d components", p->L);
-        return MG_ERR_UNSUPPORTED;
+            if (split) return lat_f64 ? mg_launch_ws_inst<KK, true, true, true> : mg_launch_ws_inst<KK, false, true, true>;
+            return lat_f64 ? mg_launch_ws_inst<KK, true, true, false> : mg_launch_ws_inst<KK, false, true, false>;
+        }
+        return nullptr;
     }
-    if (split)
-        return lat_f64 ? mg_launch_ws_inst<KK, true, false, true>(p, g, lat, out, nullptr, a, buf_bytes, lds, grid, ev)
-                       : mg_launch_ws_inst<KK, false, false, true>(p, g, lat, out, nullptr, a, buf_bytes, lds, grid, ev);
-    return lat_f64 ? mg_launch_ws_inst<KK, true, false, false>(p, g, lat, out, nullptr, a, buf_bytes, lds, grid, ev)
-                   : mg_launch_ws_inst<KK, false, false, false>(p, g, lat, out, nullptr, a, buf_bytes, lds, grid, ev);
-}
-
-int mg_launch_frames_ws(mg_primitive *p, const mg_time_grid *g, const void *lat, float *out, float *logp, const mg_frames_args &a, bool lat_f64,
-                        bool split, int buf_bytes, int lds, int grid, const mg_launch_events &ev) {
+    if (split) return lat_f64 ? mg_launch_ws_inst<KK, true, false, true> : mg_launch_ws_inst<KK, false, false, true>;
+    return lat_f64 ? mg_launch_ws_inst<KK, true, false, false> : mg_launch_ws_inst<KK, false, false, false>;
+}
+
+mg_frames_launch_fn mg_frames_ws_instance(const mg_primitive *p, bool fuse, bool lat_f64, bool split) {
+    mg_frames_launch_fn fn = nullptr;
     switch (p->KK) {
-        case 2: return mg_launch_ws_kk<2>(p, g, lat, out, logp, a, lat_f64, split, buf_bytes, lds, grid, ev);
-        case 4: return mg_launch_ws_kk<4>(p, g, lat, out, logp, a, lat_f64, split, buf_bytes, lds, grid, ev);
-        case 6: return mg_launch_ws_kk<6>(p, g, lat, out, logp, a, lat_f64, split, buf_bytes, lds, grid, ev);
-        case 8: return mg_launch_ws_kk<8>(p, g, lat, out, logp, a, lat_f64, split, buf_bytes, lds, grid, ev);
-        case 10: return mg_launch_ws_kk<10>(p, g, lat, out, logp, a, lat_f64, split, buf_bytes, lds, grid, ev);
-        case 12: return mg_launch_ws_kk<12>(p, g, lat, out, logp, a, lat_f64, split, buf_bytes, lds, grid, ev);
-        case 14: return mg_launch_ws_kk<14>(p, g, lat, out, logp, a, lat_f64, split, buf_bytes, lds, grid, ev);
-        case 16: return mg_launch_ws_kk<16>(p, g, lat, out, logp, a, lat_f64, split, buf_bytes, lds, grid, ev);
-        default: mg_set_error("mg_back_project_frames: MFMA path needs n_components <= 64"); return MG_ERR_UNSUPPORTED;
+        case 2: fn = mg_ws_inst_kk<2>(fuse, lat_f64, split); break;
+        case 4: fn = mg_ws_inst_kk<4>(fuse, lat_f64, split); break;
+        case 6: fn = mg_ws_inst_kk<6>(fuse, lat_f64, split); break;
+        case 8: fn = mg_ws_inst_kk<8>(fuse, lat_f64, split); break;
+        case 10: fn = mg_ws_inst_kk<10>(fuse, lat_f64, split); break;
+        case 12: fn = mg_ws_inst_kk<12>(fuse, lat_f64, split); break;
+        case 14: fn = mg_ws_inst_kk<14>(fuse, lat_f64, split); break;
+        case 16: fn = mg_ws_inst_kk<16>(fuse, lat_f64, split); break;
+        default: mg_set_error("mg_back_project_frames: MFMA path needs n_components <= 64"); return nullptr;
     }
+    if (!fn) mg_set_error("mg_step_frames_and_logp: no fused kernel for %d components", p->L);
+    return fn;
 }
 
 template <int KK>
diff --git a/morphablegraphs_amd/csrc/mg_host.hip b/morphablegraphs_amd/csrc/mg_host.hip
--- a/morphablegraphs_amd/csrc/mg_host.hip
+++ b/morphablegraphs_amd/csrc/mg_host.hip
@@ -8,6 +8,7 @@
 #include <time.h>
 
 #include "mg_internal.h"
+#include "mg_wait.h"
 #include <dlfcn.h>
 
 static thread_local char g_err[1024] = "";
@@ -286,15 +287,35 @@
     return nrc == 0 ? MG_OK : mg_rccl_fail(nrc, "ncclCommDestroy");
 }
 
+#define MG_WAIT_SAVED_US 6
+#define MG_WAIT_POLL_NS (100L * MG_WAIT_SAVED_US * 1000L)
+int mg_stream_wait(mg_context *ctx) {
+    const hipStream_t st = ctx->stream;
+    const hipError_t stream_state = (hipError_t)mg_poll_wait(
+        [st] {
+            const hipError_t q = hipStreamQuery(st);
+            if (q == hipErrorNotReady) (void)hipGetLastError();
+            return (int)q;
+        },
+        [] {
+            struct timespec t;
+            clock_gettime(CLOCK_MONOTONIC, &t);
+            return (int64_t)t.tv_sec * 1000000000L + t.tv_nsec;
+        },
+        [st] { return (int)hipStreamSynchronize(st); }, (int)hipErrorNotReady, MG_WAIT_POLL_NS, 16);
+    MG_HIP_CHECK(stream_state);
+    return MG_OK;
+}
+
 extern "C" int mg_context_synchronize(mg_context *ctx) {
     MG_REQUIRE(ctx != nullptr, "mg_context_synchronize: ctx is NULL");
-    MG_HIP_CHECK(hipStreamSynchronize(ctx->stream));
-    return MG_OK;
+    return mg_stream_wait(ctx);
 }
 
 extern "C" int mg_context_set_reserved_cus(mg_context *ctx, int32_t n) {
     MG_REQUIRE(ctx != nullptr && n >= 0, "mg_context_set_reserved_cus: bad arguments");
     ctx->reserved_cus = std::min<int32_t>(n, ctx->n_cu - 1);
+    ctx->launch_gen++;
     return MG_OK;
 }
 extern "C" int mg_context_set_option(mg_context *ctx, int32_t option, int32_t value) {
@@ -302,6 +323,7 @@
     MG_REQUIRE(option >= 0 && option < MG_OPT_COUNT, "mg_context_set_option: unknown option %d", option);
     MG_REQUIRE(value >= 0, "mg_context_set_option: value %d < 0", value);
     ctx->opt[option] = value;
+    ctx->launch_gen++;
     return MG_OK;
 }
 extern "C" int mg_context_device_info(mg_context *ctx, char *name, int32_t *n_cu, int64_t *total_mem) {
@@ -393,12 +415,13 @@
     MG_REQUIRE(ctx && (bytes == 0 || (dst && src)) && bytes >= 0, "mg_memcpy_h2d: bad arguments");
     if (bytes == 0) return MG_OK;
     MG_HIP_CHECK(hipMemcpyAsync(dst, src, (size_t)bytes, hipMemcpyHostToDevice, ctx->stream));
-    MG_HIP_CHECK(hipStreamSynchronize(ctx->stream));
-    return MG_OK;
-}
+    return mg_stream_wait(ctx);
+}
+static int mg_read_back_pinned(mg_context *ctx, void *dst, const void *src_dev, size_t bytes);
 extern "C" int mg_memcpy_d2h(mg_context *ctx, void *dst, const void *src, int64_t bytes) {
     MG_REQUIRE(ctx && (bytes == 0 || (dst && src)) && bytes >= 0, "mg_memcpy_d2h: bad arguments");
     if (bytes == 0) return MG_OK;
+    if ((size_t)bytes <= std::max<size_t>(ctx->pinned_bytes, MG_PINNED_MIN_BYTES)) return mg_read_back_pinned(ctx, dst, src, (size_t)bytes);
     MG_HIP_CHECK(hipMemcpyAsync(dst, src, (size_t)bytes, hipMemcpyDeviceToHost, ctx->stream));
     MG_HIP_CHECK(hipStreamSynchronize(ctx->stream));
     return MG_OK;
@@ -772,6 +795,7 @@
     for (void *q : ptrs) mg_dev_free(p->ctx, q);
     for (mg_time_grid *g : {p->canonical, p->coeff_grid})
         if (g) { mg_free_grid_device(g); delete g; }
+    mg_frames_cache_drop(p);
     delete p;
 }
 
@@ -2010,7 +2034,7 @@
         MG_HIP_CHECK(hipStreamSynchronize(ctx->stream));
         if (ctx->pinned) (void)hipHostFree(ctx->pinned);
         ctx->pinned = nullptr; ctx->pinned_bytes = 0;
-        const size_t cap = std::max<size_t>(bytes, 64 * 1024);
+        const size_t cap = std::max<size_t>(bytes, MG_PINNED_MIN_BYTES);
         MG_HIP_CHECK(hipHostMalloc(&ctx->pinned, cap, hipHostMallocDefault));
         memset(ctx->pinned, 0, cap);
         ctx->pinned_bytes = cap;
@@ -2055,7 +2079,7 @@
 static int mg_read_back_pinned(mg_context *ctx, void *dst, const void *src_dev, size_t bytes) {
     { int rcp = mg_ctx_pinned(ctx, bytes); if (rcp != MG_OK) return rcp; }
     MG_HIP_CHECK(hipMemcpyAsync(ctx->pinned, src_dev, bytes, hipMemcpyDeviceToHost, ctx->stream));
-    MG_HIP_CHECK(hipStreamSynchronize(ctx->stream));
+    { int rcw = mg_stream_wait(ctx); if (rcw != MG_OK) return rcw; }
     memcpy(dst, ctx->pinned, bytes);
     return MG_OK;
 }
diff --git a/morphablegraphs_amd/csrc/mg_internal.h b/morphablegraphs_amd/csrc/mg_internal.h
--- a/morphablegraphs_amd/csrc/mg_internal.h
+++ b/morphablegraphs_amd/csrc/mg_internal.h
@@ -51,6 +51,7 @@
     std::vector<hipEvent_t> free_events;
     int reserved_cus = 0;
     int32_t opt[MG_OPT_COUNT] = {0};
+    uint64_t launch_gen = 0;
     int prof_interval = 1;
     int64_t prof_seen[MG_PROFILE_SLOTS] = {0};
     double prof_ms[MG_PROFILE_SLOTS] = {0};
@@ -112,6 +113,8 @@
 void mg_dev_free(mg_context *ctx, void *p);
 
 int mg_ctx_scratch(mg_context *ctx, int64_t bytes, void **out);
+int mg_stream_wait(mg_context *ctx);
+#define MG_PINNED_MIN_BYTES ((size_t)64 * 1024)
 void mg_prof_begin(mg_context *ctx, int slot);
 bool mg_prof_kernel(mg_context *ctx, int slot, int slot2, hipEvent_t *start, hipEvent_t *stop);
 void mg_prof_end(mg_context *ctx, int slot);
@@ -203,6 +206,7 @@
     double *d_gchol = nullptr;
     mg_time_grid *canonical = nullptr;
     mg_time_grid *coeff_grid = nullptr;
+    struct mg_step_cache *step_cache = nullptr;
 };
 
 struct mg_constraint_set {
@@ -256,6 +260,7 @@
 
 int mg_launch_frames_mfma(mg_primitive *p, const mg_time_grid *g, const void *lat, int ldt, int64_t B, int64_t ld, float *out, float *logp,
                           int prof_slot = -1, int prof_slot2 = -1);
+void mg_frames_cache_drop(mg_primitive *p);
 bool mg_frames_can_fuse_gmm(const mg_primitive *p, const mg_time_grid *g, int64_t B);
 int mg_frames_kernel_choice(const mg_primitive *p, const mg_time_grid *g, int64_t B, bool fused, const void *out = nullptr, bool lat_f64 = false);
 int mg_output_class(mg_context *ctx, const void *p);
diff --git a/morphablegraphs_amd/csrc/mg_placement.hip b/morphablegraphs_amd/csrc/mg_placement.hip
--- a/morphablegraphs_amd/csrc/mg_placement.hip
+++ b/morphablegraphs_amd/csrc/mg_placement.hip
@@ -223,6 +223,7 @@
             if (!released) { (void)hipStreamSynchronize(ctx->stream); released = true; }
             mg_region_release(ctx, ctx->out_regions[i]);
             ctx->out_regions.erase(ctx->out_regions.begin() + (long)i);
+            ctx->launch_gen++;
         }
     mg_context::out_region r;
     int rc = mg_region_create(ctx, need, (size_t)bytes, max_candidates, &r);
@@ -244,6 +245,7 @@
     r.live = 1;
     if (info) { info[0] = r.probed; info[1] = r.ratio; info[2] = r.us; info[3] = r.fast ? 1.0 : 0.0; }
     ctx->out_regions.push_back(std::move(r));
+    ctx->launch_gen++;
     return MG_OK;
 }
 
@@ -275,6 +277,7 @@
 void mg_output_release_all(mg_context *ctx) {
     for (auto &r : ctx->out_regions) mg_region_release(ctx, r);
     ctx->out_regions.clear();
+    ctx->launch_gen++;
 }
 
 extern "C" int mg_context_trim_outputs(mg_context *ctx) {
@@ -285,6 +288,7 @@
         if (ctx->out_regions[i].live == 0) {
             mg_region_release(ctx, ctx->out_regions[i]);
             ctx->out_regions.erase(ctx->out_regions.begin() + (long)i);
+            ctx->launch_gen++;
         }
     return MG_OK;
 }
diff --git a/morphablegraphs_amd/csrc/mg_wait.h b/morphablegraphs_amd/csrc/mg_wait.h
--- /dev/null
+++ b/morphablegraphs_amd/csrc/mg_wait.h
@@ -0,0 +1,25 @@
+#pragma once
+#include <cstdint>
+
+#if defined(__x86_64__) || defined(__i386__)
+#define MG_CPU_RELAX() __builtin_ia32_pause()
+#else
+#define MG_CPU_RELAX() ((void)0)
+#endif
+
+template <class Query, class Clock, class Block>
+static inline int mg_poll_wait(Query query, Clock now_ns, Block block, int not_ready, int64_t bound_ns, unsigned polls_per_clock) {
+    int64_t t0 = 0;
+    bool have_t0 = false;
+    unsigned polls = 0;
+    for (;;) {
+        const int q = query();
+        if (q != not_ready) return q;
+        MG_CPU_RELAX();
+        if (++polls < polls_per_clock) continue;
+        polls = 0;
+        const int64_t t = now_ns();
+        if (!have_t0) { t0 = t; have_t0 = true; continue; }
+        if (t - t0 > bound_ns) return block();
+    }
+}
```

Result: no change. 110.2 million samples/s (median of 4 runs) (+0.2%).
